# octavian-ganea/equidock_public

Hardware: NVIDIA H100
Metric: protein_pairs_per_sec_iegmn_fwd_kabsch (higher is better)
Workload: dtype f32

## Files before the change

### equidock_public_b200/_native.py

```python
from __future__ import annotations

import ctypes as C
import os

_HERE = os.path.dirname(os.path.abspath(__file__))
LIB_PATH = os.environ.get('EQD_LIB_PATH') or os.path.join(_HERE, 'libeqd_iegmn.so')

ABI_VERSION = 14
EDGE_FEATS, N_RBF, HID, H0, H0_PAD, N_RES_TYPES, HEADS, TILE_ROWS = 27, 15, 64, 69, 72, 21, 50, 128
STATUS_SVD_DEGENERATE, STATUS_NAN, STATUS_DEGREE_OVERFLOW, STATUS_BAD_RESIDUE = 1, 2, 4, 8

_vp, _i32, _f32 = C.c_void_p, C.c_int32, C.c_float


class EqdGraph(C.Structure):
    _fields_ = [('n_pairs', _i32), ('n_nodes', _i32), ('n_lig_nodes', _i32), ('n_edges', _i32),
                ('n_lig_edges', _i32), ('max_in_degree', _i32),
                ('seg_ptr', _vp), ('row_ptr', _vp), ('col_src', _vp), ('edge_dst', _vp),
                ('he_lig', _vp), ('he_rec', _vp),
                ('n_node_tiles', _i32), ('node_tiles', _vp)]


class EqdLayerParams(C.Structure):
    _fields_ = [('dh', _i32), ('dhp', _i32),
                ('w_proj', _vp), ('b_proj', _vp), ('w_edge1', _vp), ('edge_ln_g', _vp), ('edge_ln_b', _vp),
                ('w_edge2', _vp), ('b_edge2', _vp), ('w_coor1', _vp), ('b_coor1', _vp), ('w_coor2', _vp),
                ('b_coor2', _f32), ('w_edge_tc', _vp), ('w_node_tc', _vp), ('w_proj_tc', _vp),
                ('w_node1', _vp), ('b_node1', _vp), ('node_ln_g', _vp), ('node_ln_b', _vp),
                ('w_node2', _vp), ('b_node2', _vp),
                ('skip_weight_h', _f32), ('x_connection_init', _f32), ('leaky_slope', _f32), ('mma_products', _i32)]


class EqdLayerConsts(C.Structure):
    _fields_ = [('edge', _f32 * 64 * 5), ('node', _f32 * 304), ('proj_bias', _f32 * 320)]


class EqdDropout(C.Structure):
    _fields_ = [('seed', C.c_uint64), ('p', _f32), ('scale', _f32), ('threshold', C.c_uint32), ('layer', _i32),
                ('rank', _i32), ('reserved', _i32)]


def dropout_descriptor(p: float, seed: int, layer: int, rank: int = 0) -> EqdDropout:
    import numpy as np
    d = EqdDropout()
    d.seed, d.p, d.layer, d.rank = int(seed) & 0xFFFFFFFFFFFFFFFF, float(p), int(layer), int(rank)
    d.threshold = min(int(round(float(p) * 2.0 ** 32)), 0xFFFFFFFF)
    d.scale = 0.0 if p >= 1.0 else float(np.float32(1.0 / (1.0 - float(p))))
    return d


class EqdLayer(C.Structure):
    _fields_ = [('dev', EqdLayerParams), ('consts', EqdLayerConsts), ('dropout', EqdDropout)]


class EqdForwardIO(C.Structure):
    _fields_ = [(n, _vp) for n in ('emb', 'res_lig', 'res_rec', 'mu_lig', 'mu_rec', 'x_lig', 'x_rec', 'rot', 'trans',
                                   'ligand_out', 'sing', 'status', 'h_out', 'x_out', 'keypts', 'cov', 'ymean', 'stage_events',
                                   'train_stash')] + \
               [('train_stash_bytes', C.c_size_t)]


class EqdHeadParams(C.Structure):
    _fields_ = [('w_mean', _vp), ('b_mean', _vp), ('w_key', _vp), ('w_query', _vp), ('m_qk', _vp), ('leaky_slope', _f32)]


class EqdPairArchive(C.Structure):
    _fields_ = [('n_pairs', _i32)] + [(n, _vp) for n in (
        'lig_node_ptr', 'rec_node_ptr', 'lig_edge_ptr', 'rec_edge_ptr', 'pocket_ptr', 'lig_res_feat', 'rec_res_feat',
        'lig_x', 'rec_x', 'lig_mu_r_norm', 'rec_mu_r_norm', 'lig_src', 'lig_dst', 'rec_src', 'rec_dst', 'lig_he', 'rec_he',
        'lig_new_x', 'pocket_coors', 'bound_lig', 'bound_rec', 'lig_centroid')]


class EqdBatchOut(C.Structure):
    _fields_ = [(n, _vp) for n in ('res_feat', 'x', 'new_x', 'mu_r_norm', 'row_ptr', 'col_src', 'edge_dst', 'he_lig', 'he_rec',
                                   'seg_ptr',
                                   'node_tiles', 'pocket_ptr', 'pocket_lig', 'pocket_rec', 'bound_lig', 'bound_rec', 'rot',
                                   'trans')]


_G, _L, _H = C.POINTER(EqdGraph), C.POINTER(EqdLayer), C.POINTER(EqdHeadParams)
PROTOTYPES = {
    'eqd_abi_version': (C.c_int, []),
    'eqd_workspace_bytes': (C.c_size_t, [_i32, _i32, _i32]),
    'eqd_embed': (C.c_int, [_G, _vp, _vp, _vp, _vp, _vp, _vp, _vp, _vp, _vp, _vp]),
    'eqd_embed_checked': (C.c_int, [_G, _vp, _vp, _vp, _vp, _vp, _vp, _vp, _vp, _vp, _vp, _vp]),
    'eqd_project': (C.c_int, [_G, _L, _vp, _i32, _vp, _vp]),
    'eqd_edge_stage': (C.c_int, [_G, _L, _vp, _vp, _vp, _vp, _vp, _vp, _vp]),
    'eqd_edge_stage_ffma': (C.c_int, [_G, _L, _vp, _vp, _vp, _vp, _vp, _vp, _vp]),
    'eqd_node_stage': (C.c_int, [_G, _L, _L, _vp, _i32, _vp, _vp, _vp, _vp, _vp, _vp, _vp]),
    'eqd_kv_blocks_bytes': (C.c_size_t, [_i32]),
    'eqd_project_tc': (C.c_int, [_G, _L, _vp, _vp, _vp, _vp]),
    'eqd_project_tc0': (C.c_int, [_G, _L, _vp, _vp, _vp, _vp, _vp]),
    'eqd_attention_tc0': (C.c_int, [_G, _vp, _vp, _vp, _vp, _vp]),
    'eqd_node_mlp_tc0': (C.c_int, [_G, _L, _vp, _vp, _vp, _vp, _vp]),
    'eqd_node_stage_tc0': (C.c_int, [_G, _L, _L, _vp, _vp, _vp, _vp, _vp, _vp, _vp, _vp, _vp]),
    'eqd_kv_blocks': (C.c_int, [_G, _vp, _i32, _i32, _i32, _vp, _vp]),
    'eqd_attention_tc': (C.c_int, [_G, _vp, _vp, _vp, _vp]),
    'eqd_node_mlp_tc': (C.c_int, [_G, _L, _vp, _vp, _vp, _vp, _vp, _vp]),
    'eqd_node_stage_tc': (C.c_int, [_G, _L, _L, _vp, _vp, _vp, _vp, _vp, _vp, _vp, _vp, _vp]),
    'eqd_iegmn_layer_forward': (C.c_int, [_G, _L, _L, _vp, _i32, _vp, _vp, _vp, _vp, _vp, _vp, _vp, _vp, _vp, _vp,
                                          _vp]),
    'eqd_head_fold': (C.c_int, [_H, _vp, _vp]),
    'eqd_forward_workspace_bytes': (C.c_size_t, [_G]),
    'eqd_iegmn_forward': (C.c_int, [_G, C.POINTER(_L), _i32, _H, C.POINTER(EqdForwardIO), _vp, C.c_size_t, _vp]),
    'eqd_forward_stash_bytes': (C.c_size_t, [_G, _i32]),
    'eqd_forward_stash_offsets': (C.c_int, [_G, _i32, C.POINTER(C.c_size_t)]),
    'eqd_tn_partial_floats': (C.c_size_t, [C.c_int64, _i32, _i32, C.POINTER(_i32), C.POINTER(_i32)]),
    'eqd_tn_gemm': (C.c_int, [_vp, _i32, _i32, _vp, _i32, _i32, C.c_int64, _f32, _vp, _vp, C.POINTER(_i32), _vp]),
    'eqd_grad_reduce': (C.c_int, [_vp, _i32, C.c_int64, _vp, _vp, _i32, _vp, _vp]),
    'eqd_bwd_node_mlp': (C.c_int, [_G, _L] + [_vp] * 3 + [_i32, _vp, _vp, _i32] + [_vp] * 9 + [C.POINTER(_i32), _vp]),
    'eqd_bwd_attention': (C.c_int, [_G, _L, _vp, _vp, _i32, _vp, _vp, _vp, _vp]),
    'eqd_bwd_edge': (C.c_int, [_G, _L] + [_vp] * 14 + [C.POINTER(_i32), _vp]),
    'eqd_bwd_edge_gather': (C.c_int, [_G, _vp, _vp, _vp, _vp, _vp, _f32, _vp, _i32, _vp, _vp]),
    'eqd_bwd_project': (C.c_int, [_G, _L, _vp, _vp, _vp, _vp]),
    'eqd_bwd_embed': (C.c_int, [_G, _vp, _vp, _vp, _vp, _vp, _vp]),
    'eqd_bwd_head_workspace_bytes': (C.c_size_t, [_i32, _i32, _i32]),
    'eqd_bwd_head': (C.c_int, [_G, _H] + [_vp] * 9 + [C.c_size_t] + [_vp] * 6),
    'eqd_bwd_head_dropout': (C.c_int, [_G, _H, C.POINTER(EqdDropout)] + [_vp] * 9 + [C.c_size_t] + [_vp] * 6),
    'eqd_bwd_layer_inputs': (C.c_int, [_G, _L] + [_vp] * 5),
    'eqd_bwd_inputs': (C.c_int, [_G] + [_vp] * 11),
    'eqd_losses_workspace_bytes': (C.c_size_t, [_i32, _i32]),
    'eqd_losses': (C.c_int, [_G] + [_vp] * 7 + [_i32, _i32, _f32, _f32, _f32, _f32, _vp, C.c_size_t] + [_vp] * 6),
    'eqd_graph_build_workspace_bytes': (C.c_size_t, [_i32]),
    'eqd_graph_build_knn': (C.c_int, [_i32, _i32, _i32, _vp, _vp, _vp, _vp, _vp, _f32, _i32, _vp, C.c_size_t, _vp, _vp, _vp, _vp]),
    'eqd_graph_build_edges': (C.c_int, [_i32, _vp, _vp, _vp, _vp, _vp, _vp, _vp]),
    'eqd_assemble_batch': (C.c_int, [C.POINTER(EqdPairArchive), _i32, _vp, _i32, C.c_uint64, C.c_uint64, _i32, _f32, _i32,
                                     C.POINTER(EqdBatchOut), _vp]),
    'eqd_rmsd_meter': (C.c_int, [_G, _vp, _vp, _vp, _vp, _vp, _vp]),
    'eqd_sqnorm_partials': (C.c_int, [_vp, C.c_int64, _vp, _i32, _vp]),
    'eqd_clip_adam': (C.c_int, [_vp, _vp, _vp, _vp, C.c_int64, _vp, _i32, _f32, _f32, _f32, _f32, _f32, _f32, _i32, _f32, _vp, _vp]),
    'eqd_event_create': (_vp, []),
    'eqd_event_destroy': (None, [_vp]),
    'eqd_event_elapsed_ms': (C.c_float, [_vp, _vp]),
    'eqd_keypoints': (C.c_int, [_G, _H, _vp, _vp, _vp, C.c_size_t, _vp, _vp, _vp, _vp]),
    'eqd_keypoints_dropout': (C.c_int, [_G, _H, C.POINTER(EqdDropout), _vp, _vp, _vp, C.c_size_t, _vp, _vp, _vp, _vp]),
    'eqd_kabsch_apply': (C.c_int, [_G, _vp, _vp, _vp, _vp, _vp, _vp, _vp, _vp, _vp, _vp]),
}

_lib = None


class NativeLibraryError(RuntimeError):
    pass


def load():
    global _lib
    if _lib is not None:
        return _lib
    if not os.path.isfile(LIB_PATH):
        raise NativeLibraryError(
            f'{LIB_PATH} not found: build it with equidock_public_b200/csrc/build.sh '
            '(python -c "import __graft_entry__ as g; g.build()"). This engine has no CPU fallback.')
    lib = C.CDLL(LIB_PATH)
    for name, (res, args) in PROTOTYPES.items():
        fn = getattr(lib, name)
        fn.restype, fn.argtypes = res, args
    if lib.eqd_abi_version() != ABI_VERSION:
        raise NativeLibraryError(f'ABI mismatch: library {lib.eqd_abi_version()} vs binding {ABI_VERSION}')
    _lib = lib
    return lib


def check(rc: int, what: str):
    if rc == 0:
        return
    if rc <= -1000:
        raise NativeLibraryError(f'{what}: CUDA error {-(rc + 1000)} at kernel launch')
    names = {-1: 'EQD_ERR_BAD_ARG', -2: 'EQD_ERR_UNSUPPORTED', -3: 'EQD_ERR_WORKSPACE'}
    raise NativeLibraryError(f'{what}: {names.get(rc, rc)}')


def ptr(t):
    if t is None:
        return None
    return C.c_void_p(t.data_ptr())
```

### equidock_public_b200/csrc/edge_stage_tc.cu

```cuda
#include "tc_common.cuh"

namespace eqd {
#define TC_WGS 3
#define TC_THREADS (128 * TC_WGS)
#define TC_ROWS 64
#define TC_MAX_TN 32
#define TC_LD 72
#define TC_W_BYTES 67584
#define TC_W1_SPLIT 6144
#define TC_W23_BASE 18432
#define TC_W23_SPLIT 16384
#define TC_HE_FLOATS (TC_ROWS * EQD_EDGE_FEATS + 16)
#define TC_A_SPLIT 6144

struct __align__(128) TcWgSmem {
  unsigned char a[3 * TC_A_SPLIT];
  float msg[TC_ROWS * TC_LD];
  float he[TC_HE_FLOATS];
  double xs[2][TC_ROWS * 6];
  double xm[TC_ROWS * 3];
  double phi[TC_ROWS];
  int src[2][TC_ROWS];
  int dst[2][TC_ROWS];
  int rp[2][TC_MAX_TN + 4];
  unsigned long long he_bar;
};

struct EdgeConsts {
  float ln_g[64], ln_b[64], b2[64], b3[64], w4[64];
};

struct TcSmem {
  unsigned char w[TC_W_BYTES];
  TcWgSmem wg[TC_WGS];
  EdgeConsts cst;
  unsigned long long w_bar;
};

template <int P>
__global__ void __launch_bounds__(TC_THREADS, 1)
edge_stage_tc_kernel(eqd_graph g, eqd_layer_params p, const __grid_constant__ EdgeConsts cst_p,
                     const float* __restrict__ proj, const double* __restrict__ x_in, const double* __restrict__ x_orig,
                     float* __restrict__ aggr, double* __restrict__ x_out, int* __restrict__ status, int tn) {
  extern __shared__ __align__(128) unsigned char smem_raw[];
  TcSmem& S = *reinterpret_cast<TcSmem*>(smem_raw);
  const int tid = threadIdx.x, wgi = tid >> 7, t = tid & 127, r = t & 63, half = t >> 6;
  const int warp = t >> 5, lane = t & 31;
  TcWgSmem& W = S.wg[wgi];
  const EdgeConsts& cst = S.cst;
  const int bar = 1 + wgi;
  const int pw = 128 + 3 * p.dhp;
  const int ntiles = (g.n_nodes + tn - 1) / tn;
  const float slope = p.leaky_slope;

  if (tid == 0) {
    mbar_init(&S.w_bar, 1);
    for (int w = 0; w < TC_WGS; ++w) mbar_init(&S.wg[w].he_bar, 1);
    asm volatile("fence.mbarrier_init.release.cluster;" ::: "memory");
    mbar_expect_tx(&S.w_bar, TC_W_BYTES);
    bulk_g2s(S.w, p.w_edge_tc, TC_W_BYTES, &S.w_bar);
  }
  for (int i = tid; i < 5 * 64; i += TC_THREADS) (&S.cst.ln_g[0])[i] = (&cst_p.ln_g[0])[i];
  __syncthreads();
  mbar_wait(&S.w_bar, 0);
  unsigned he_phase = 0;
  const unsigned w_saddr = smem_u32(S.w), a_saddr = smem_u32(W.a);
  auto a_desc = [&](int sp, int kb) { return a_desc_at<TC_ROWS>(a_saddr, TC_A_SPLIT, 0, sp, kb); };

  auto prefetch = [&](int tile, int buf, int e0, int e1, int& off_l, int& n_l, int& off_r) {
    const int n0 = tile * tn, nn = min(tn, g.n_nodes - n0);
    const int ne = e1 - e0;
    off_l = off_r = 0;
    n_l = 0;
    if (ne <= TC_ROWS) {
      if (r < ne) {
        if (half == 0) cp_async4(&W.src[buf][r], g.col_src + e0 + r);
        else cp_async4(&W.dst[buf][r], g.edge_dst + e0 + r);
      }
      if (half == 0 && r <= nn) cp_async4(&W.rp[buf][r], g.row_ptr + n0 + r);
      const int el0 = min(e0, g.n_lig_edges), el1 = min(e1, g.n_lig_edges);
      n_l = el1 - el0;
      long sl = 0, sr = 0;
      unsigned bl = 0, br = 0;
      if (n_l > 0) {
        long b0 = (long)el0 * (EQD_EDGE_FEATS * 4), b1 = (long)el1 * (EQD_EDGE_FEATS * 4);
        sl = b0 & ~15L;
        bl = (unsigned)(((b1 + 15) & ~15L) - sl);
        off_l = (int)((b0 - sl) >> 2);
      }
      const int nr = ne - n_l;
      const unsigned dst_r_off = bl;
      if (nr > 0) {
        long b0 = (long)(e0 + n_l - g.n_lig_edges) * (EQD_EDGE_FEATS * 4), b1 = (long)(e1 - g.n_lig_edges) * (EQD_EDGE_FEATS * 4);
        sr = b0 & ~15L;
        br = (unsigned)(((b1 + 15) & ~15L) - sr);
        off_r = (int)(dst_r_off >> 2) + (int)((b0 - sr) >> 2);
      }
      if (t == 0) {
        mbar_expect_tx(&W.he_bar, bl + br);
        if (bl) bulk_g2s(W.he, reinterpret_cast<const unsigned char*>(g.he_lig) + sl, bl, &W.he_bar);
        if (br) bulk_g2s(reinterpret_cast<unsigned char*>(W.he) + dst_r_off, reinterpret_cast<const unsigned char*>(g.he_rec) + sr, br,
                         &W.he_bar);
      }
    }
    cp_async_commit();
  };
  auto prefetch_x = [&](int b, int ne_t) {
    if (r < ne_t && ne_t <= TC_ROWS) {
      const double* xp = x_in + (long)(half == 0 ? W.src[b][r] : W.dst[b][r]) * 3;
#pragma unroll
      for (int c = 0; c < 3; ++c) cp_async8(&W.xs[b][r * 6 + half * 3 + c], xp + c);
    }
    cp_async_commit();
  };
  auto row_range = [&](int tile, int& e0, int& e1) {
    const int n0 = tile * tn;
    e0 = __ldg(g.row_ptr + n0);
    e1 = __ldg(g.row_ptr + n0 + min(tn, g.n_nodes - n0));
  };

  int tile = blockIdx.x * TC_WGS + wgi;
  const int tstride = gridDim.x * TC_WGS;
  int buf = 0;
  int e0 = 0, ne = 0, off_l = 0, n_l = 0, off_r = 0;
  if (tile < ntiles) {
    int e1;
    row_range(tile, e0, e1);
    ne = e1 - e0;
    prefetch(tile, buf, e0, e1, off_l, n_l, off_r);
    cp_async_wait<0>();
    prefetch_x(buf, ne);
  }
  const int fr0 = warp * 16 + (lane >> 2), fc = 2 * (lane & 3);

  for (; tile < ntiles; tile += tstride) {
    const int n0 = tile * tn, nn = min(tn, g.n_nodes - n0);
    const bool has_next = tile + tstride < ntiles;
    int e0n = 0, e1n = 0, off_ln = 0, n_ln = 0, off_rn = 0;
    if (has_next) row_range(tile + tstride, e0n, e1n);
    const int nen = e1n - e0n;
    if (ne > TC_ROWS) {
      if (t == 0) atomicOr(status + g.n_pairs, EQD_STATUS_DEGREE_OVERFLOW);
      cp_async_wait<0>();
      wg_barrier(bar);
      if (has_next) {
        prefetch(tile + tstride, buf ^ 1, e0n, e1n, off_ln, n_ln, off_rn);
        cp_async_wait<0>();
        prefetch_x(buf ^ 1, nen);
      }
      e0 = e0n; ne = nen; off_l = off_ln; n_l = n_ln; off_r = off_rn; buf ^= 1;
      continue;
    }
    const int o_upd = 127 - t;
    const int nd_upd = o_upd / 3, comp_upd = o_upd - nd_upd * 3;
    const long gi_upd = (long)(n0 + nd_upd) * 3 + comp_upd;
    double xo_upd = 0.0, xi_upd = 0.0;
    if (o_upd < nn * 3) {
      xo_upd = x_orig[gi_upd];
      xi_upd = x_in[gi_upd];
    }
    cp_async_wait<0>();
    wg_barrier(bar);
    float2 ps[16], pd[16];
#pragma unroll
    for (int h = 0; h < 2; ++h) {
      const int fr = fr0 + 8 * h;
      const bool ok = fr < ne;
      const float* sp = proj + (long)(ok ? W.src[buf][fr] : 0) * pw + fc;
      const float* dp = proj + (long)(ok ? W.dst[buf][fr] : n0) * pw + 64 + fc;
#pragma unroll
      for (int j = 0; j < 8; ++j) {
        ps[2 * j + h] = __ldg(reinterpret_cast<const float2*>(sp + 8 * j));
        pd[2 * j + h] = __ldg(reinterpret_cast<const float2*>(dp + 8 * j));
      }
    }
    const bool valid = r < ne;
    {
      float a1v[24];
      mbar_wait(&W.he_bar, he_phase);
      he_phase ^= 1;
      const float* hrow = W.he + (r < n_l ? off_l + r * EQD_EDGE_FEATS : off_r + (r - n_l) * EQD_EDGE_FEATS);
      if (half == 0) {
#pragma unroll
        for (int k = 0; k < 24; ++k) a1v[k] = valid ? hrow[k] : 0.f;
      } else {
        double rx = 0.0, ry = 0.0, rz = 0.0;
        if (valid) {
          const double* xs = W.xs[buf] + r * 6;
          rx = xs[0] - xs[3];
          ry = xs[1] - xs[4];
          rz = xs[2] - xs[5];
          W.xm[r * 3 + 0] = rx;
          W.xm[r * 3 + 1] = ry;
          W.xm[r * 3 + 2] = rz;
        }
#pragma unroll
        for (int k = 0; k < 3; ++k) a1v[k] = valid ? hrow[24 + k] : 0.f;
        const float nd2 = valid ? -(float)(rx * rx + ry * ry + rz * rz) : -INFINITY;
        constexpr double kS[EQD_N_RBF] = {1.0, 1.5, 2.25, 3.375, 5.0625, 7.59375, 11.390625, 17.0859375, 25.62890625,
                                          38.443359375, 57.6650390625, 86.49755859375, 129.746337890625,
                                          194.6195068359375, 291.92926025390625};
#pragma unroll
        for (int j = 0; j < EQD_N_RBF; ++j)
          a1v[3 + j] = exp2f(nd2 * (float)(1.4426950408889634 / kS[j]));
#pragma unroll
        for (int k = 18; k < 24; ++k) a1v[k] = 0.f;
      }
      unsigned p0[12], p1[12], p2[12];
#pragma unroll
      for (int c = 0; c < 12; ++c) split3_pair<P>(a1v[2 * c], a1v[2 * c + 1], p0[c], p1[c], p2[c]);
#pragma unroll
      for (int j = 0; j < 3; ++j) a_store8<TC_ROWS, P>(W.a, TC_A_SPLIT, r, half * 24 + 8 * j, p0 + 4 * j, p1 + 4 * j, p2 + 4 * j);
    }
    tc_fence_before();
    const bool deg10 = wg_barrier_and(bar, t >= nn || W.rp[buf][t + 1] - W.rp[buf][t] == 10);
    unsigned af[3][4][4];
    {
      float v[32];
      wg_gemm6_issue<64, 0, P>(v, a_desc, [&](int sp, int kb) { return b_desc_ex(w_saddr + sp * TC_W1_SPLIT + kb * 2048, 1024, 128); },
                         3, false);
      if (has_next) prefetch(tile + tstride, buf ^ 1, e0n, e1n, off_ln, n_ln, off_rn);
      wg_mma_wait(v);
#pragma unroll
      for (int h = 0; h < 2; ++h)
#pragma unroll
        for (int j = 0; j < 8; ++j) {
          float& x0 = v[4 * j + 2 * h];
          float& x1 = v[4 * j + 2 * h + 1];
          x0 = __fadd_rn(__fadd_rn(x0, ps[2 * j + h].x), pd[2 * j + h].x);
          x1 = __fadd_rn(__fadd_rn(x1, ps[2 * j + h].y), pd[2 * j + h].y);
          x0 = fmaxf(x0, __fmul_rn(x0, slope));
          x1 = fmaxf(x1, __fmul_rn(x1, slope));
        }
      float pv[32];
#pragma unroll
      for (int i = 0; i < 32; ++i) pv[i] = __shfl_xor_sync(0xffffffffu, v[i], 2);
      float mean[2], rstd[2];
#pragma unroll
      for (int h = 0; h < 2; ++h) {
        float mh[2], qh[2];
#pragma unroll
        for (int ch = 0; ch < 2; ++ch) {
          float s0 = 0.f, s1 = 0.f;
#pragma unroll
          for (int c4 = 0; c4 < 8; ++c4) {
            s0 = __fadd_rn(s0, chain_val(v, pv, h, ch, c4, 0));
            s1 = __fadd_rn(s1, chain_val(v, pv, h, ch, c4, 1));
          }
          const float sp = s0 + s1;
          mh[ch] = (sp + __shfl_xor_sync(0xffffffffu, sp, 1)) * (1.f / 32.f);
          float q0 = 0.f, q1 = 0.f;
#pragma unroll
          for (int c4 = 0; c4 < 8; ++c4) {
            const float d0 = __fadd_rn(chain_val(v, pv, h, ch, c4, 0), -mh[ch]);
            const float d1 = __fadd_rn(chain_val(v, pv, h, ch, c4, 1), -mh[ch]);
            q0 = fmaf(d0, d0, q0);
            q1 = fmaf(d1, d1, q1);
          }
          const float qp = q0 + q1;
          qh[ch] = qp + __shfl_xor_sync(0xffffffffu, qp, 1);
        }
        const float m0 = mh[0], m1 = mh[1];
        mean[h] = 0.5f * (m0 + m1);
        const float dm = m0 - m1;
        const float var = (qh[0] + qh[1] + dm * dm * 16.f) * (1.f / 64.f);
        rstd[h] = 1.f / sqrtf(var + 1e-5f);
      }
#pragma unroll
      for (int j = 0; j < 8; ++j) {
        const float2 gj = *reinterpret_cast<const float2*>(&cst.ln_g[8 * j + fc]);
        const float2 bj = *reinterpret_cast<const float2*>(&cst.ln_b[8 * j + fc]);
#pragma unroll
        for (int h = 0; h < 2; ++h) {
          float& x0 = v[4 * j + 2 * h];
          float& x1 = v[4 * j + 2 * h + 1];
          x0 = fmaf(__fmul_rn(__fadd_rn(x0, -mean[h]), rstd[h]), gj.x, bj.x);
          x1 = fmaf(__fmul_rn(__fadd_rn(x1, -mean[h]), rstd[h]), gj.y, bj.y);
        }
      }
      acc_to_a_split3<4, P>(v, af);
    }
    if (has_next) {
      cp_async_wait<0>();
      prefetch_x(buf ^ 1, nen);
    }
    {
      auto w23 = [&](int hn) {
        return [&, hn](int sp, int kb) {
          return b_desc_ex(w_saddr + TC_W23_BASE + sp * TC_W23_SPLIT + kb * 4096 + hn * 1024, 2048, 128); };
      };
      float m[32], hd[32];
      wg_gemm6_rs_issue<64, 4, 0, false, P>(m, af, w23(0), false);
      wg_gemm6_rs_issue<64, 4, 0, false, P>(hd, af, w23(1), false);
      wg_mma_wait(m);
      wg_mma_wait(hd);
      float u[32];
#pragma unroll
      for (int j = 0; j < 8; ++j) {
        const float2 b2 = *reinterpret_cast<const float2*>(&cst.b2[8 * j + fc]);
        const float2 b3 = *reinterpret_cast<const float2*>(&cst.b3[8 * j + fc]);
#pragma unroll
        for (int h = 0; h < 2; ++h) {
          *reinterpret_cast<float2*>(W.msg + (fr0 + 8 * h) * TC_LD + 8 * j + fc) =
              make_float2(__fadd_rn(m[4 * j + 2 * h], b2.x), __fadd_rn(m[4 * j + 2 * h + 1], b2.y));
          const float x0 = __fadd_rn(hd[4 * j + 2 * h], b3.x), x1 = __fadd_rn(hd[4 * j + 2 * h + 1], b3.y);
          u[4 * j + 2 * h] = fmaxf(x0, __fmul_rn(x0, slope));
          u[4 * j + 2 * h + 1] = fmaxf(x1, __fmul_rn(x1, slope));
        }
      }
      float pu[32];
#pragma unroll
      for (int i = 0; i < 32; ++i) pu[i] = __shfl_xor_sync(0xffffffffu, u[i], 2);
      double phv[2];
#pragma unroll
      for (int h = 0; h < 2; ++h) {
        double red[2];
#pragma unroll
        for (int ch = 0; ch < 2; ++ch) {
          const float* w4 = cst.w4 + 32 * ch + 2 * (lane & 1);
          float p0 = 0.f, p1 = 0.f;
#pragma unroll
          for (int c4 = 0; c4 < 8; ++c4) {
            p0 = fmaf(chain_val(u, pu, h, ch, c4, 0), w4[4 * c4], p0);
            p1 = fmaf(chain_val(u, pu, h, ch, c4, 1), w4[4 * c4 + 1], p1);
          }
          const double pp = (double)p0 + (double)p1;
          red[ch] = pp + __shfl_xor_sync(0xffffffffu, pp, 1);
        }
        phv[h] = red[0] + red[1] + (double)p.b_coor2;
      }
      if ((lane & 3) == 0) {
        W.phi[fr0] = phv[0];
        W.phi[fr0 + 8] = phv[1];
      }
    }
    wg_barrier(bar);
    if (o_upd < nn * 3) {
      const int rs = W.rp[buf][nd_upd] - e0, re = W.rp[buf][nd_upd + 1] - e0;
      double sum = 0.0;
      if (deg10) {
#pragma unroll
        for (int j = 0; j < 10; ++j) {
          const int rr = nd_upd * 10 + j;
          sum += W.xm[rr * 3 + comp_upd] * W.phi[rr];
        }
      } else {
        for (int rr = rs; rr < re; ++rr) sum += W.xm[rr * 3 + comp_upd] * W.phi[rr];
      }
      const int deg = re - rs;
      const double upd = deg > 0 ? sum / (double)deg : 0.0;
      const double eta = (double)p.x_connection_init;
      x_out[gi_upd] = eta * xo_upd + (1.0 - eta) * xi_upd + upd;
    }
    {
      const int c = t & 63;
      const float* col = W.msg + c;
      if (deg10) {
        for (int nd = (nn * half) >> 1, nd1 = (nn * (half + 1)) >> 1; nd < nd1; ++nd) {
          const float* cr = col + nd * 10 * TC_LD;
          float s0 = 0.f, s1 = 0.f;
#pragma unroll
          for (int j = 0; j < 10; j += 2) {
            s0 += cr[j * TC_LD];
            s1 += cr[(j + 1) * TC_LD];
          }
          aggr[(long)(n0 + nd) * 64 + c] = (s0 + s1) / 10.f;
        }
      } else {
        for (int nd = (nn * half) >> 1, nd1 = (nn * (half + 1)) >> 1; nd < nd1; ++nd) {
          const int rs = W.rp[buf][nd] - e0, re = W.rp[buf][nd + 1] - e0;
          float s0 = 0.f, s1 = 0.f;
          int rr = rs;
          for (; rr + 1 < re; rr += 2) {
            s0 += col[rr * TC_LD];
            s1 += col[(rr + 1) * TC_LD];
          }
          if (rr < re) s0 += col[rr * TC_LD];
          aggr[(long)(n0 + nd) * 64 + c] = re > rs ? (s0 + s1) / (float)(re - rs) : 0.f;
        }
      }
    }
    e0 = e0n; ne = nen; off_l = off_ln; n_l = n_ln; off_r = off_rn; buf ^= 1;
  }
  cp_async_wait<0>();
  __syncthreads();
}

template <int P>
static int launch_edge_stage_tc(const eqd_graph* g, const eqd_layer* p_l, const float* proj, const double* x_in,
                                const double* x_orig, float* aggr, double* x_out, int32_t* status, int tn, void* stream) {
  const int ntiles = (g->n_nodes + tn - 1) / tn;
  EdgeConsts cst;
  memcpy(&cst, p_l->consts.edge, sizeof(cst));
  size_t smem = sizeof(TcSmem) + 128;
  EQD_SET_SMEM((edge_stage_tc_kernel<P>), smem);
  int grid = (ntiles + TC_WGS - 1) / TC_WGS;
  if (grid > EQD_SMS) grid = EQD_SMS;
  edge_stage_tc_kernel<P><<<grid, TC_THREADS, smem, (cudaStream_t)stream>>>(*g, p_l->dev, cst, proj, x_in, x_orig, aggr,
                                                                           x_out, status, tn);
  EQD_CUDA_LAUNCH_CHECK();
  return EQD_OK;
}

}

extern "C" int eqd_edge_stage(const eqd_graph* g, const eqd_layer* p_l, const float* proj, const double* x_in,
                              const double* x_orig, float* aggr, double* x_out, int32_t* status, void* stream) {
  const eqd_layer_params* p = p_l ? &p_l->dev : nullptr;
  if (!g || !p || !proj || !x_in || !x_orig || !aggr || !x_out || !status) return EQD_ERR_BAD_ARG;
  if (!p->w_edge_tc) return EQD_ERR_BAD_ARG;
  const int products = eqd_mma_products(p);
  if (!products) return EQD_ERR_UNSUPPORTED;
  if (g->max_in_degree < 1 || g->max_in_degree > EQD_TM) return EQD_ERR_UNSUPPORTED;
  if (!(p->leaky_slope >= 0.f && p->leaky_slope <= 1.f)) return EQD_ERR_UNSUPPORTED;
  if ((reinterpret_cast<uintptr_t>(g->he_lig) | reinterpret_cast<uintptr_t>(g->he_rec) |
       reinterpret_cast<uintptr_t>(p->w_edge_tc)) & 15)
    return EQD_ERR_BAD_ARG;
  if (g->max_in_degree > TC_ROWS || p_l->dropout.p > 0.f) return eqd_edge_stage_ffma(g, p_l, proj, x_in, x_orig, aggr, x_out, status, stream);
  if (g->n_nodes <= 0) return EQD_OK;
  int tn = TC_ROWS / g->max_in_degree;
  if (tn > TC_MAX_TN) tn = TC_MAX_TN;
  return products == 3 ? eqd::launch_edge_stage_tc<3>(g, p_l, proj, x_in, x_orig, aggr, x_out, status, tn, stream)
                       : eqd::launch_edge_stage_tc<6>(g, p_l, proj, x_in, x_orig, aggr, x_out, status, tn, stream);
}
```

### equidock_public_b200/csrc/forward.cu

```cuda
#include <cstdint>

#include "common.cuh"

namespace {

inline size_t al256(size_t v) { return (v + 255) & ~(size_t)255; }

struct Carve {
  size_t h0, x0, xa, xb, ha, hb, pa, pb, aggr, mu, kv, x5, head, keypts, ymean, cov, total;
  size_t kv_bytes, x5_rows, head_bytes;
};

Carve carve(const eqd_graph* g) {
  Carve c;
  const size_t N = (size_t)(g->n_nodes > 0 ? g->n_nodes : 0), B = (size_t)(g->n_pairs > 0 ? g->n_pairs : 0);
  size_t o = 0;
  auto take = [&](size_t bytes) { size_t at = o; o += al256(bytes); return at; };
  c.h0 = take(N * EQD_H0_PAD * 4);
  c.x0 = take(N * 3 * 8);
  c.xa = take(N * 3 * 8);
  c.xb = take(N * 3 * 8);
  c.ha = take(N * EQD_HID * 4);
  c.hb = take(N * EQD_HID * 4);
  c.pa = take(N * (128 + 3 * EQD_H0_PAD) * 4);
  c.pb = take(N * (128 + 3 * EQD_H0_PAD) * 4);
  c.aggr = take(N * EQD_HID * 4);
  c.mu = take(N * EQD_H0_PAD * 4);
  c.kv_bytes = eqd_kv_blocks_bytes(g->n_nodes);
  c.kv = take(c.kv_bytes);
  c.x5_rows = ((N + 7) / 8 + 8) * 8;
  c.x5 = take(c.x5_rows * 16 * 4);
  c.head_bytes = eqd_workspace_bytes(g->n_nodes, g->n_node_tiles, g->n_pairs);
  c.head = take(c.head_bytes);
  c.keypts = take(2 * B * EQD_HEADS * 3 * 8);
  c.ymean = take(2 * B * 3 * 8);
  c.cov = take(B * 9 * 8);
  c.total = o;
  return c;
}

}

extern "C" size_t eqd_forward_workspace_bytes(const eqd_graph* g) { return g ? carve(g).total : 0; }

namespace {
struct Stash {
  size_t h0, x, h, aggr, mu, total, x_stride, h_stride, a_stride, m_stride;
};
Stash stash_layout(const eqd_graph* g, int n_layers) {
  Stash s;
  const size_t N = (size_t)(g->n_nodes > 0 ? g->n_nodes : 0), L = (size_t)(n_layers > 0 ? n_layers : 0);
  s.x_stride = al256(N * 3 * 8);
  s.h_stride = al256(N * EQD_HID * 4);
  s.a_stride = al256(N * EQD_HID * 4);
  s.m_stride = al256(N * EQD_H0_PAD * 4);
  size_t o = 0;
  s.h0 = o; o += al256(N * EQD_H0_PAD * 4);
  s.x = o; o += L * s.x_stride;
  s.h = o; o += L * s.h_stride;
  s.aggr = o; o += L * s.a_stride;
  s.mu = o; o += L * s.m_stride;
  s.total = o;
  return s;
}
}

extern "C" size_t eqd_forward_stash_bytes(const eqd_graph* g, int32_t n_layers) { return g ? stash_layout(g, n_layers).total : 0; }
extern "C" int eqd_forward_stash_offsets(const eqd_graph* g, int32_t n_layers, size_t* out ) {
  if (!g || !out) return EQD_ERR_BAD_ARG;
  const Stash s = stash_layout(g, n_layers);
  out[0] = s.h0; out[1] = s.x; out[2] = s.x_stride; out[3] = s.h; out[4] = s.h_stride; out[5] = s.aggr; out[6] = s.a_stride;
  out[7] = s.mu; out[8] = s.m_stride;
  return EQD_OK;
}

extern "C" int eqd_iegmn_forward(const eqd_graph* g, const eqd_layer* const* layers, int32_t n_layers,
                                 const eqd_head_params* hp, const eqd_forward_io* io, void* workspace,
                                 size_t workspace_bytes, void* stream) {
  if (!g || !layers || n_layers < 1 || !hp || !io || !workspace) return EQD_ERR_BAD_ARG;
  if (!io->emb || !io->res_lig || !io->res_rec || !io->mu_lig || !io->mu_rec || !io->x_lig || !io->x_rec || !io->rot ||
      !io->trans || !io->ligand_out || !io->sing || !io->status || !io->h_out || !io->x_out)
    return EQD_ERR_BAD_ARG;
  if ((reinterpret_cast<uintptr_t>(io->h_out) | reinterpret_cast<uintptr_t>(io->x_out)) & 15)
    return EQD_ERR_BAD_ARG;
  for (int li = 0; li < n_layers; ++li)
    if (!layers[li]) return EQD_ERR_BAD_ARG;
  const Carve c = carve(g);
  if (workspace_bytes < c.total) return EQD_ERR_WORKSPACE;
  if (reinterpret_cast<uintptr_t>(workspace) & 255) return EQD_ERR_BAD_ARG;
  if (g->n_pairs <= 0 || g->n_nodes <= 0) return EQD_OK;
  cudaStream_t st = (cudaStream_t)stream;
  unsigned char* w = reinterpret_cast<unsigned char*>(workspace);
  float* h0 = reinterpret_cast<float*>(w + c.h0);
  double* x0 = reinterpret_cast<double*>(w + c.x0);
  double* xbuf[2] = {reinterpret_cast<double*>(w + c.xa), reinterpret_cast<double*>(w + c.xb)};
  float* hbuf[2] = {reinterpret_cast<float*>(w + c.ha), reinterpret_cast<float*>(w + c.hb)};
  float* pa = reinterpret_cast<float*>(w + c.pa);
  float* pb = reinterpret_cast<float*>(w + c.pb);
  float* aggr = reinterpret_cast<float*>(w + c.aggr);
  float* mu = reinterpret_cast<float*>(w + c.mu);
  unsigned char* kv = w + c.kv;
  float* x5 = reinterpret_cast<float*>(w + c.x5);
  double* keypts = io->keypts ? io->keypts : reinterpret_cast<double*>(w + c.keypts);
  double* ymean = io->ymean ? io->ymean : reinterpret_cast<double*>(w + c.ymean);
  double* cov = io->cov ? io->cov : reinterpret_cast<double*>(w + c.cov);
  const int N = g->n_nodes, B = g->n_pairs;
  unsigned char* sb = reinterpret_cast<unsigned char*>(io->train_stash);
  Stash sl;
  if (sb) {
    sl = stash_layout(g, n_layers);
    if (io->train_stash_bytes < sl.total || (reinterpret_cast<uintptr_t>(sb) & 255)) return EQD_ERR_WORKSPACE;
    h0 = reinterpret_cast<float*>(sb + sl.h0);
    x0 = reinterpret_cast<double*>(sb + sl.x);
  }

  const size_t plane = c.kv_bytes / 6, from = (size_t)(N / 8) * 1024;
  cudaError_t me = cudaSuccess;
  for (int pl = 0; pl < 6 && me == cudaSuccess; ++pl) me = cudaMemsetAsync(kv + pl * plane + from, 0, plane - from, st);
  if (me == cudaSuccess) me = cudaMemsetAsync(x5 + (size_t)N * 16, 0, (c.x5_rows - (size_t)N) * 16 * 4, st);
  if (me == cudaSuccess) me = cudaMemsetAsync(io->status, 0, (size_t)(B + 1) * sizeof(int32_t), st);
  if (me != cudaSuccess) return -(1000 + (int)me);
  auto stage_event = [&](int li, int which) {
    if (io->stage_events && io->stage_events[li * 4 + which]) cudaEventRecord((cudaEvent_t)io->stage_events[li * 4 + which], st);
  };
  int rc = eqd_embed_checked(g, io->emb, io->res_lig, io->res_rec, io->mu_lig, io->mu_rec, io->x_lig, io->x_rec, h0, x0,
                             io->status, stream);
  if (rc) return rc;
  const eqd_layer* l0_l = layers[0];
  const eqd_layer_params* l0 = &l0_l->dev;
  bool drop = false;
  for (int li = 0; li < n_layers; ++li) drop = drop || layers[li]->dropout.p > 0.f;
  const bool tc0 = l0->dh == EQD_H0 && l0->w_proj_tc && l0->w_node_tc && !drop;
  if (tc0) rc = eqd_project_tc0(g, l0_l, h0, pa, kv, x5, stream);
  else rc = eqd_project(g, l0_l, h0, l0->dh == EQD_H0 ? EQD_H0_PAD : EQD_HID, pa, stream);
  if (rc) return rc;
  const float* h_in = h0;
  int ldh = l0->dh == EQD_H0 ? EQD_H0_PAD : EQD_HID;
  const double* x_in = x0;
  for (int li = 0; li < n_layers; ++li) {
    const eqd_layer* lp_l = layers[li];
    const eqd_layer* lpn_l = li + 1 < n_layers ? layers[li + 1] : nullptr;
    const eqd_layer_params* lp = &lp_l->dev;
    const eqd_layer_params* lpn = lpn_l ? &lpn_l->dev : nullptr;
    const bool last = lpn == nullptr;
    float* h_out = last ? io->h_out : hbuf[li & 1];
    double* x_out = last ? io->x_out : xbuf[li & 1];
    if (sb) {
      if (!last) {
        h_out = reinterpret_cast<float*>(sb + sl.h + (size_t)(li + 1) * sl.h_stride);
        x_out = reinterpret_cast<double*>(sb + sl.x + (size_t)(li + 1) * sl.x_stride);
      }
      aggr = reinterpret_cast<float*>(sb + sl.aggr + (size_t)li * sl.a_stride);
      mu = reinterpret_cast<float*>(sb + sl.mu + (size_t)li * sl.m_stride);
    }
    stage_event(li, 0);
    rc = eqd_edge_stage(g, lp_l, pa, x_in, x0, aggr, x_out, io->status, stream);
    if (rc) return rc;
    stage_event(li, 1);
    stage_event(li, 2);
    if (lp->dh == EQD_HID && lp->w_node_tc && !drop && (!lpn || lpn->w_proj_tc)) {
      rc = eqd_node_stage_tc(g, lp_l, lpn_l, h_in, h0, pa, aggr, kv, mu, h_out, pb, stream);
    } else if (li == 0 && tc0 && (!lpn || lpn->w_proj_tc)) {
      rc = eqd_node_stage_tc0(g, lp_l, lpn_l, h0, pa, aggr, kv, x5, mu, h_out, pb, stream);
    } else {
      rc = eqd_node_stage(g, lp_l, lpn_l, h_in, ldh, h0, pa, aggr, sb ? mu : nullptr, h_out, pb, stream);
      if (!rc && lpn && lpn->dh == EQD_HID && lpn->w_node_tc && !drop) rc = eqd_kv_blocks(g, pb, 320, 192, 256, kv, stream);
    }
    if (rc) return rc;
    stage_event(li, 3);
    float* t = pa; pa = pb; pb = t;
    h_in = h_out;
    ldh = EQD_HID;
    x_in = x_out;
  }
  eqd_dropout head_drop = layers[n_layers - 1]->dropout;
  head_drop.layer = n_layers;
  rc = eqd_keypoints_dropout(g, hp, &head_drop, h_in, x_in, w + c.head, c.head_bytes, keypts, ymean, cov, stream);
  if (rc) return rc;
  return eqd_kabsch_apply(g, cov, ymean, io->x_lig, nullptr, io->rot, io->trans, io->ligand_out, io->sing, io->status, stream);
}

extern "C" void* eqd_event_create(void) {
  cudaEvent_t e = nullptr;
  return cudaEventCreate(&e) == cudaSuccess ? (void*)e : nullptr;
}
extern "C" void eqd_event_destroy(void* e) {
  if (e) cudaEventDestroy((cudaEvent_t)e);
}
extern "C" float eqd_event_elapsed_ms(void* a, void* b) {
  float ms = -1.f;
  if (!a || !b || cudaEventElapsedTime(&ms, (cudaEvent_t)a, (cudaEvent_t)b) != cudaSuccess) return -1.f;
  return ms;
}
```

### equidock_public_b200/csrc/node_mlp_tc.cu

```cuda
#include "tc_common.cuh"

namespace eqd {

#define NM_THREADS 256
#define NM_W5_SPLIT 34816
#define NM_W6_BASE 104448
#define NM_W6_SPLIT 8192
#define NM_W_BYTES 129024

struct NmConsts { float b5[64], ln_g[64], ln_b[64], b6[64]; };

#define NM_CHAINS 2
#define NM_SLOTS 3

struct NmSmem {
  unsigned char w[NM_W_BYTES];
  float stage[NM_CHAINS][NM_SLOTS][64 * 64];
  float c[256];
  unsigned long long w_bar;
};

template <int P>
__global__ void __launch_bounds__(NM_CHAINS * 128, 1)
node_mlp_tc_kernel(int n_nodes, eqd_layer_params p, const __grid_constant__ NmConsts cst, const float* __restrict__ h_in,
                   const float* __restrict__ aggr, const float* __restrict__ mu, const float* __restrict__ h0,
                   float* __restrict__ h_out) {
  extern __shared__ __align__(128) unsigned char smem_raw[];
  NmSmem& S = *reinterpret_cast<NmSmem*>(smem_raw);
  const int tid = threadIdx.x, wgi = tid >> 7, t = tid & 127, lane = t & 31;
  float (&ring)[NM_SLOTS][64 * 64] = S.stage[wgi];
  const int bar = 1 + wgi;
  const int ntiles = (n_nodes + 63) / 64, tstride = gridDim.x * NM_CHAINS, tile0 = blockIdx.x * NM_CHAINS + wgi;
  if (tid == 0) {
    mbar_init(&S.w_bar, 1);
    asm volatile("fence.mbarrier_init.release.cluster;" ::: "memory");
    mbar_expect_tx(&S.w_bar, NM_W_BYTES);
    bulk_g2s(S.w, p.w_node_tc, NM_W_BYTES, &S.w_bar);
  }
  for (int i = tid; i < 256; i += NM_CHAINS * 128) S.c[i] = reinterpret_cast<const float*>(&cst)[i];
  __syncthreads();
  const unsigned w_saddr = smem_u32(S.w);
  const float slope = p.leaky_slope, sk = p.skip_weight_h, sk1 = 1.f - p.skip_weight_h;
  const int fr0 = (t >> 5) * 16 + (lane >> 2), fc = 2 * (lane & 3);

  auto issue = [&](int q) {
    const int tile = tile0 + (q >> 2) * tstride, pc = q & 3;
    if (tile < ntiles) {
      const float* src = pc == 0 ? h_in : pc == 1 ? aggr : pc == 2 ? mu : h0;
      stage_rows64(ring[q % NM_SLOTS], src, pc == 3 ? EQD_H0_PAD : EQD_HID, 0, (long)tile * 64, min(64, n_nodes - tile * 64), t);
    } else {
      cp_async_commit();
    }
  };
  int q = 0;
  for (int i = 0; i < NM_SLOTS - 1; ++i) issue(i);
  mbar_wait(&S.w_bar, 0);

  for (int tile = tile0; tile < ntiles; tile += tstride) {
    const int node0 = tile * 64, nvalid = min(64, n_nodes - node0);
    float2 x4[2];
#pragma unroll
    for (int hh = 0; hh < 2; ++hh) {
      const int row = fr0 + 8 * hh;
      x4[hh] = row < nvalid ? *reinterpret_cast<const float2*>(h0 + (long)(node0 + row) * EQD_H0_PAD + 64 + fc)
                            : make_float2(0.f, 0.f);
    }
    float acc[32], hs[32];
#pragma unroll
    for (int j = 0; j < 8; ++j) {
      const float2 bj = *reinterpret_cast<const float2*>(&S.c[8 * j + fc]);
#pragma unroll
      for (int hh = 0; hh < 2; ++hh) {
        acc[4 * j + 2 * hh] = bj.x;
        acc[4 * j + 2 * hh + 1] = bj.y;
      }
    }
#pragma unroll 1
    for (int pc = 0; pc < 4; ++pc, ++q) {
      cp_async_wait<NM_SLOTS - 2>();
      wg_barrier(bar);
      issue(q + NM_SLOTS - 1);
      float v[32];
      staged_rows_to_frag(ring[q % NM_SLOTS], t, v);
      if (pc == 0) {
#pragma unroll
        for (int i = 0; i < 32; ++i) hs[i] = v[i];
      }
      unsigned af[3][4][4];
      acc_to_a_split3<4, P>(v, af);
      float d[32];
      wg_gemm6_rs_issue<64, 4, 0, false, P>(d, af, [&](int sp, int kb) {
        return b_desc_ex(w_saddr + (4 * pc + kb) * 2048 + sp * NM_W5_SPLIT, 1024, 128); }, false);
      wg_mma_wait(d);
#pragma unroll
      for (int i = 0; i < 32; ++i) acc[i] = __fadd_rn(acc[i], d[i]);
    }
    {
      unsigned a4[3][1][4];
#pragma unroll
      for (int hh = 0; hh < 2; ++hh) split3_pair<P>(x4[hh].x, x4[hh].y, a4[0][0][hh], a4[1][0][hh], a4[2][0][hh]);
#pragma unroll
      for (int sp = 0; sp < 3; ++sp) a4[sp][0][2] = a4[sp][0][3] = 0u;
      float d[32];
      wg_gemm6_rs_issue<64, 1, 0, false, P>(d, a4, [&](int sp, int kb) {
        return b_desc_ex(w_saddr + 16 * 2048 + sp * NM_W5_SPLIT, 1024, 128); }, false);
      wg_mma_wait(d);
#pragma unroll
      for (int i = 0; i < 32; ++i) acc[i] = __fadd_rn(acc[i], d[i]);
    }
    unsigned af[3][4][4];
    {
      float (&v)[32] = acc;
#pragma unroll
      for (int i = 0; i < 32; ++i) v[i] = fmaxf(v[i], __fmul_rn(v[i], slope));
      float pv[32];
#pragma unroll
      for (int i = 0; i < 32; ++i) pv[i] = __shfl_xor_sync(0xffffffffu, v[i], 2);
      float msum[2], rstd[2];
#pragma unroll
      for (int h = 0; h < 2; ++h) {
        float mh[2], qh[2];
#pragma unroll
        for (int ch = 0; ch < 2; ++ch) {
          float s0 = 0.f, s1 = 0.f;
#pragma unroll
          for (int c4 = 0; c4 < 8; ++c4) {
            s0 = __fadd_rn(s0, chain_val(v, pv, h, ch, c4, 0));
            s1 = __fadd_rn(s1, chain_val(v, pv, h, ch, c4, 1));
          }
          const float sp = __fadd_rn(s0, s1);
          mh[ch] = __fmul_rn(__fadd_rn(sp, __shfl_xor_sync(0xffffffffu, sp, 1)), 1.f / 32.f);
          float q0 = 0.f, q1 = 0.f;
#pragma unroll
          for (int c4 = 0; c4 < 8; ++c4) {
            const float d0 = __fadd_rn(chain_val(v, pv, h, ch, c4, 0), -mh[ch]);
            const float d1 = __fadd_rn(chain_val(v, pv, h, ch, c4, 1), -mh[ch]);
            q0 = __fmaf_rn(d0, d0, q0);
            q1 = __fmaf_rn(d1, d1, q1);
          }
          const float qp = __fadd_rn(q0, q1);
          qh[ch] = __fadd_rn(qp, __shfl_xor_sync(0xffffffffu, qp, 1));
        }
        msum[h] = __fadd_rn(mh[0], mh[1]);
        const float dm = __fadd_rn(mh[0], -mh[1]);
        const float var = __fmaf_rn(__fmul_rn(dm, dm), 16.f, __fadd_rn(qh[0], qh[1]));
        rstd[h] = 1.f / sqrtf(__fmaf_rn(var, 1.f / 64.f, 1e-5f));
      }
#pragma unroll
      for (int j = 0; j < 8; ++j) {
        const float2 gj = *reinterpret_cast<const float2*>(&S.c[64 + 8 * j + fc]);
        const float2 bj = *reinterpret_cast<const float2*>(&S.c[128 + 8 * j + fc]);
#pragma unroll
        for (int h = 0; h < 2; ++h) {
          float& x0 = v[4 * j + 2 * h];
          float& x1 = v[4 * j + 2 * h + 1];
          x0 = __fmaf_rn(__fmul_rn(__fmaf_rn(msum[h], -0.5f, x0), rstd[h]), gj.x, bj.x);
          x1 = __fmaf_rn(__fmul_rn(__fmaf_rn(msum[h], -0.5f, x1), rstd[h]), gj.y, bj.y);
        }
      }
      acc_to_a_split3<4, P>(v, af);
    }
    {
      float d[32];
      wg_gemm6_rs_issue<64, 4, 0, false, P>(d, af, [&](int sp, int kb) {
        return b_desc_ex(w_saddr + NM_W6_BASE + sp * NM_W6_SPLIT + kb * 2048, 1024, 128); }, false);
      wg_mma_wait(d);
#pragma unroll
      for (int hh = 0; hh < 2; ++hh) {
        const int row = fr0 + 8 * hh;
        if (row < nvalid) {
          float* o = h_out + (long)(node0 + row) * EQD_HID + fc;
#pragma unroll
          for (int j = 0; j < 8; ++j) {
            const float2 bj = *reinterpret_cast<const float2*>(&S.c[192 + 8 * j + fc]);
            const int i = 4 * j + 2 * hh;
            *reinterpret_cast<float2*>(o + 8 * j) =
                make_float2(__fmaf_rn(__fadd_rn(d[i], bj.x), sk, __fmul_rn(hs[i], sk1)),
                            __fmaf_rn(__fadd_rn(d[i + 1], bj.y), sk, __fmul_rn(hs[i + 1], sk1)));
          }
        }
      }
    }
  }
  cp_async_wait<0>();
}


#define NM0_W5_SPLIT 35840
#define NM0_W6_BASE 107520
#define NM0_W6_SPLIT 10240
#define NM0_W_BYTES 138240
#define NM0_A_SPLIT 20480
#define NM0_LD 84

struct Nm0Consts { float b5[80], ln_g[80], ln_b[80], b6[64]; };

struct Nm0Smem {
  unsigned char w[NM0_W_BYTES];
  unsigned char a[3 * NM0_A_SPLIT];
  float red[EQD_TM * 4];
  unsigned long long w_bar;
};

__global__ void __launch_bounds__(NM_THREADS, 1)
node_mlp0_tc_kernel(int n_nodes, eqd_layer_params p, const __grid_constant__ Nm0Consts cst, const float* __restrict__ h0,
                    const float* __restrict__ aggr, const float* __restrict__ mu , float* __restrict__ h_out) {
  extern __shared__ __align__(128) unsigned char smem_raw[];
  Nm0Smem& S = *reinterpret_cast<Nm0Smem*>(smem_raw);
  const int tid = threadIdx.x, q = tid, half = q >> 7, r = q & 127, wgi = tid >> 7;
  const int ntiles = (n_nodes + EQD_TM - 1) / EQD_TM;
  if (tid == 0) {
    mbar_init(&S.w_bar, 1);
    asm volatile("fence.mbarrier_init.release.cluster;" ::: "memory");
    mbar_expect_tx(&S.w_bar, NM0_W_BYTES);
    bulk_g2s(S.w, p.w_node_tc, NM0_W_BYTES, &S.w_bar);
  }
  __syncthreads();
  const unsigned w_saddr = smem_u32(S.w), a_saddr = smem_u32(S.a);
  float* const dtile = reinterpret_cast<float*>(S.a);
  auto a_desc = [&](int sp, int kb) { return a_desc_at<EQD_TM>(a_saddr, NM0_A_SPLIT, wgi, sp, kb); };
  mbar_wait(&S.w_bar, 0);
  const float slope = p.leaky_slope;
  float* red = S.red;

  for (int tile = blockIdx.x; tile < ntiles; tile += gridDim.x) {
    const int node = tile * EQD_TM + r;
    const bool valid = node < n_nodes;
    auto row32 = [&](const float* base, int ld, float (&v)[32]) {
      const float4* sp = reinterpret_cast<const float4*>(base + (long)node * ld + half * 32);
#pragma unroll
      for (int c4 = 0; c4 < 8; ++c4) {
        float4 t = valid ? sp[c4] : make_float4(0.f, 0.f, 0.f, 0.f);
        v[c4 * 4] = t.x; v[c4 * 4 + 1] = t.y; v[c4 * 4 + 2] = t.z; v[c4 * 4 + 3] = t.w;
      }
    };
    auto extra8 = [&](const float* base) {
      if (half == 0) {
        const float4* ep = reinterpret_cast<const float4*>(base + (long)node * EQD_H0_PAD + 64);
        float4 a = valid ? ep[0] : make_float4(0.f, 0.f, 0.f, 0.f), b = valid ? ep[1] : make_float4(0.f, 0.f, 0.f, 0.f);
        float t[8] = {a.x, a.y, a.z, a.w, b.x, b.y, b.z, b.w};
        store_extra8_split3<EQD_TM>(S.a, NM0_A_SPLIT, r, 64, t);
      }
    };
    float acc[32], accx[16];
#pragma unroll
    for (int c = 0; c < 32; ++c) acc[c] = cst.b5[half * 32 + c];
#pragma unroll
    for (int c = 0; c < 16; ++c) accx[c] = cst.b5[64 + c];
    auto piece = [&](int kb0, int nkb) {
      tc_fence_before();
      __syncthreads();
      {
        float d[40];
        wg_gemm6<80>(d, a_desc, [&](int sp, int kb) {
          return b_desc_ex(w_saddr + (kb0 + kb) * (80 * 32) + sp * NM0_W5_SPLIT, 80 * 16, 128); }, nkb, false);
        __syncthreads();
        wg_store_d<80>(dtile + wgi * 64 * NM0_LD, NM0_LD, d, tid & 127);
      }
      __syncthreads();
      const float* dr = dtile + r * NM0_LD;
#pragma unroll
      for (int c = 0; c < 32; ++c) acc[c] += dr[half * 32 + c];
      if (half == 0) {
#pragma unroll
        for (int c = 0; c < 16; ++c) accx[c] += dr[64 + c];
      }
      __syncthreads();
    };
    {
      float v[32];
      row32(h0, EQD_H0_PAD, v);
      store_half_split3<EQD_TM>(S.a, NM0_A_SPLIT, r, half * 32, v);
      extra8(h0);
      piece(0, 5);
      row32(aggr, EQD_HID, v);
      store_half_split3<EQD_TM>(S.a, NM0_A_SPLIT, r, half * 32, v);
      piece(5, 4);
      row32(mu, EQD_H0_PAD, v);
      store_half_split3<EQD_TM>(S.a, NM0_A_SPLIT, r, half * 32, v);
      extra8(mu);
      piece(9, 5);
    }
    {
      const int nh = half == 0 ? 37 : 32;
      float sum = 0.f;
#pragma unroll
      for (int c = 0; c < 32; ++c) {
        acc[c] = lrelu(acc[c], slope);
        sum += acc[c];
      }
      if (half == 0) {
#pragma unroll
        for (int c = 0; c < 5; ++c) {
          accx[c] = lrelu(accx[c], slope);
          sum += accx[c];
        }
      }
      const float mh = sum / (float)nh;
      float m2 = 0.f;
#pragma unroll
      for (int c = 0; c < 32; ++c) {
        float d = acc[c] - mh;
        m2 = fmaf(d, d, m2);
      }
      if (half == 0) {
#pragma unroll
        for (int c = 0; c < 5; ++c) {
          float d = accx[c] - mh;
          m2 = fmaf(d, d, m2);
        }
      }
      red[(r * 2 + half) * 2 + 0] = mh;
      red[(r * 2 + half) * 2 + 1] = m2;
      __syncthreads();
      const float m0 = red[r * 4 + 0], m1 = red[r * 4 + 2];
      const float mean = (37.f * m0 + 32.f * m1) * (1.f / 69.f);
      const float dm = m0 - m1;
      const float var = (red[r * 4 + 1] + red[r * 4 + 3] + dm * dm * (37.f * 32.f / 69.f)) * (1.f / 69.f);
      const float rstd = 1.f / sqrtf(var + 1e-5f);
#pragma unroll
      for (int c = 0; c < 32; ++c) acc[c] = (acc[c] - mean) * rstd * cst.ln_g[half * 32 + c] + cst.ln_b[half * 32 + c];
      store_half_split3<EQD_TM>(S.a, NM0_A_SPLIT, r, half * 32, acc);
      if (half == 0) {
        float t[8];
#pragma unroll
        for (int c = 0; c < 5; ++c) t[c] = (accx[c] - mean) * rstd * cst.ln_g[64 + c] + cst.ln_b[64 + c];
        t[5] = t[6] = t[7] = 0.f;
        store_extra8_split3<EQD_TM>(S.a, NM0_A_SPLIT, r, 64, t);
      }
    }
    tc_fence_before();
    __syncthreads();
    {
      float d[32];
      wg_gemm6<64>(d, a_desc, [&](int sp, int kb) {
        return b_desc_ex(w_saddr + NM0_W6_BASE + sp * NM0_W6_SPLIT + kb * 2048, 1024, 128); }, 5, false);
      __syncthreads();
      wg_store_d<64>(dtile + wgi * 64 * NM0_LD, NM0_LD, d, tid & 127);
    }
    __syncthreads();
    {
      float v[32];
      tile_ld32f(dtile, NM0_LD, r, half * 32, v);
#pragma unroll
      for (int c = 0; c < 32; ++c) v[c] += cst.b6[half * 32 + c];
      if (valid) {
        float4* o = reinterpret_cast<float4*>(h_out + (long)node * EQD_HID + half * 32);
#pragma unroll
        for (int c4 = 0; c4 < 8; ++c4) o[c4] = make_float4(v[c4 * 4], v[c4 * 4 + 1], v[c4 * 4 + 2], v[c4 * 4 + 3]);
      }
    }
    __syncthreads();
  }
}

template <int P>
static int launch_node_mlp_tc(const eqd_graph* g, const eqd_layer* p_l, const float* h_in, const float* aggr,
                              const float* mu, const float* h0, float* h_out, void* stream) {
  NmConsts cst;
  memcpy(&cst, p_l->consts.node, sizeof(cst));
  const int ntiles = (g->n_nodes + 63) / 64;
  const size_t smem = sizeof(NmSmem) + 128;
  EQD_SET_SMEM(node_mlp_tc_kernel<P>, smem);
  int grid = (ntiles + NM_CHAINS - 1) / NM_CHAINS;
  if (grid > EQD_SMS) grid = EQD_SMS;
  node_mlp_tc_kernel<P><<<grid, NM_CHAINS * 128, smem, (cudaStream_t)stream>>>(g->n_nodes, p_l->dev, cst, h_in, aggr, mu,
                                                                             h0, h_out);
  EQD_CUDA_LAUNCH_CHECK();
  return EQD_OK;
}

}

extern "C" int eqd_node_mlp_tc(const eqd_graph* g, const eqd_layer* p_l, const float* h_in, const float* aggr,
                               const float* mu, const float* h0, float* h_out, void* stream) {
  const eqd_layer_params* p = p_l ? &p_l->dev : nullptr;
  if (!g || !p || !h_in || !aggr || !mu || !h0 || !h_out) return EQD_ERR_BAD_ARG;
  if (p_l->dropout.p > 0.f) return EQD_ERR_UNSUPPORTED;
  if (p->dh != 64 || p->dhp != 64) return EQD_ERR_UNSUPPORTED;
  if (!(p->leaky_slope >= 0.f && p->leaky_slope <= 1.f)) return EQD_ERR_UNSUPPORTED;
  const int products = eqd_mma_products(p);
  if (!products) return EQD_ERR_UNSUPPORTED;
  if (!p->w_node_tc || (reinterpret_cast<uintptr_t>(p->w_node_tc) & 15)) return EQD_ERR_BAD_ARG;
  if (g->n_nodes <= 0) return EQD_OK;
  return products == 3 ? eqd::launch_node_mlp_tc<3>(g, p_l, h_in, aggr, mu, h0, h_out, stream)
                       : eqd::launch_node_mlp_tc<6>(g, p_l, h_in, aggr, mu, h0, h_out, stream);
}

extern "C" int eqd_node_mlp_tc0(const eqd_graph* g, const eqd_layer* p_l, const float* h0, const float* aggr,
                                const float* mu, float* h_out, void* stream) {
  const eqd_layer_params* p = p_l ? &p_l->dev : nullptr;
  if (!g || !p || !h0 || !aggr || !mu || !h_out) return EQD_ERR_BAD_ARG;
  if (p_l->dropout.p > 0.f) return EQD_ERR_UNSUPPORTED;
  if (p->dh != 69 || p->dhp != 72 || !eqd_mma_products(p)) return EQD_ERR_UNSUPPORTED;
  if (!(p->leaky_slope >= 0.f && p->leaky_slope <= 1.f)) return EQD_ERR_UNSUPPORTED;
  if (!p->w_node_tc || (reinterpret_cast<uintptr_t>(p->w_node_tc) & 15)) return EQD_ERR_BAD_ARG;
  if (g->n_nodes <= 0) return EQD_OK;
  eqd::Nm0Consts cst;
  memcpy(&cst, p_l->consts.node, sizeof(cst));
  int ntiles = (g->n_nodes + EQD_TM - 1) / EQD_TM;
  size_t smem = sizeof(eqd::Nm0Smem) + 128;
  EQD_SET_SMEM((eqd::node_mlp0_tc_kernel), smem);
  int grid = ntiles < EQD_SMS ? ntiles : EQD_SMS;
  eqd::node_mlp0_tc_kernel<<<grid, NM_THREADS, smem, (cudaStream_t)stream>>>(g->n_nodes, *p, cst, h0, aggr, mu, h_out);
  EQD_CUDA_LAUNCH_CHECK();
  return EQD_OK;
}

extern "C" int eqd_attention_tc0(const eqd_graph*, const float*, const void*, const float*, float*, void*);

extern "C" int eqd_node_stage_tc0(const eqd_graph* g, const eqd_layer* p_l, const eqd_layer* p_next_l,
                                  const float* h0, const float* proj, const float* aggr, void* kv, const float* x5,
                                  float* mu, float* h_out, float* proj_next, void* stream) {
  const eqd_layer_params* p = p_l ? &p_l->dev : nullptr;
  const eqd_layer_params* p_next = p_next_l ? &p_next_l->dev : nullptr;
  if (!g || !p || !kv || !mu || !x5) return EQD_ERR_BAD_ARG;
  if (p_next && !proj_next) return EQD_ERR_BAD_ARG;
  if (!eqd_mma_products(p)) return EQD_ERR_UNSUPPORTED;
  int rc = eqd_attention_tc0(g, proj, kv, x5, mu, stream);
  if (rc) return rc;
  rc = eqd_node_mlp_tc0(g, p_l, h0, aggr, mu, h_out, stream);
  if (rc) return rc;
  if (p_next) rc = eqd_project_tc(g, p_next_l, h_out, proj_next, kv, stream);
  return rc;
}

extern "C" int eqd_project_tc(const eqd_graph*, const eqd_layer*, const float*, float*, void*, void*);
int eqd_attention_tc_products(const eqd_graph*, const float*, const void*, float*, int, void*);


extern "C" int eqd_node_stage_tc(const eqd_graph* g, const eqd_layer* p_l, const eqd_layer* p_next_l,
                                 const float* h_in, const float* h0, const float* proj, const float* aggr, void* kv,
                                 float* mu, float* h_out, float* proj_next, void* stream) {
  const eqd_layer_params* p = p_l ? &p_l->dev : nullptr;
  const eqd_layer_params* p_next = p_next_l ? &p_next_l->dev : nullptr;
  if (!g || !p || !kv || !mu) return EQD_ERR_BAD_ARG;
  if (p_next && !proj_next) return EQD_ERR_BAD_ARG;
  const int products = eqd_mma_products(p);
  if (!products) return EQD_ERR_UNSUPPORTED;
  int rc = eqd_attention_tc_products(g, proj, kv, mu, products, stream);
  if (rc) return rc;
  rc = eqd_node_mlp_tc(g, p_l, h_in, aggr, mu, h0, h_out, stream);
  if (rc) return rc;
  if (p_next) rc = eqd_project_tc(g, p_next_l, h_out, proj_next, kv, stream);
  return rc;
}
```

### equidock_public_b200/engine.py

```python
from __future__ import annotations

import ctypes as C
import sys
import threading
from typing import Dict, List, Optional, Sequence

import numpy as np
import torch

from . import _native as nat
from .hetero_graph import LIGAND, LL, RECEPTOR, RR


def _dev_f32(t, device):
    return t.detach().to(device=device, dtype=torch.float32).contiguous()


def _host_f32(t):
    return t.detach().to(device='cpu', dtype=torch.float32).contiguous()


def _upload_blob(tensors: Dict[str, torch.Tensor], device) -> Dict[str, torch.Tensor]:
    offs, total = {}, 0
    for k, t in tensors.items():
        offs[k] = total
        total += (t.numel() * t.element_size() + 255) & ~255
    host = torch.zeros(max(total, 256), dtype=torch.uint8)
    for k, t in tensors.items():
        n = t.numel() * t.element_size()
        host[offs[k]:offs[k] + n] = t.contiguous().view(-1).view(torch.uint8)
    dev = host.to(device)
    out = {}
    for k, t in tensors.items():
        n = t.numel() * t.element_size()
        out[k] = dev[offs[k]:offs[k] + n].view(t.dtype).view(t.shape)
    out['_blob'] = dev
    return out


def umma_bf16x3(w: torch.Tensor) -> torch.Tensor:
    n, k = w.shape
    assert n % 8 == 0 and k % 8 == 0
    parts, r = [], w.to(torch.float32)
    for _ in range(3):
        b = r.to(torch.bfloat16)
        parts.append(b)
        r = r - b.to(torch.float32)
    out = [b.reshape(n // 8, 8, k // 8, 8).permute(2, 0, 1, 3).contiguous().reshape(-1) for b in parts]
    return torch.cat(out)


_PY_FORWARD = False

PRECISIONS = {'fp32': 0, 'bf16x3': 3}


def draw_dropout(p: float, rank: int = 0):
    if not p > 0:
        return None
    seed = int(torch.empty((), dtype=torch.int64).random_(-2 ** 63, 2 ** 63 - 1)) & 0xFFFFFFFFFFFFFFFF
    return float(p), seed, int(rank)


def with_dropout(descs, dropout, first_layer: int = 0):
    if dropout is None:
        return list(descs)
    p, seed, rank = dropout
    out = []
    for li, d in enumerate(descs):
        c = nat.EqdLayer.from_buffer_copy(d)
        c.dropout = nat.dropout_descriptor(p, seed, first_layer + li, rank)
        out.append(c)
    return out


def head_dropout(dropout, n_layers: int):
    return None if dropout is None else nat.dropout_descriptor(dropout[0], dropout[1], n_layers, dropout[2])


def check_precision(precision: str) -> str:
    if precision not in PRECISIONS:
        raise ValueError(f'precision must be one of {sorted(PRECISIONS)}, got {precision!r}')
    return precision


class PackedLayer:

    def __init__(self, sd: Dict[str, torch.Tensor], device, skip_weight_h: float, x_connection_init: float,
                 leaky_slope: float):
        f = lambda k: _host_f32(sd[k])
        w1, b1 = f('edge_mlp.0.weight'), f('edge_mlp.0.bias')
        wq, wk, wv = f('att_mlp_Q.0.weight'), f('att_mlp_K.0.weight'), f('att_mlp_V.0.weight')
        w5, b5 = f('node_mlp.0.weight'), f('node_mlp.0.bias')
        w6, b6 = f('node_mlp.4.weight'), f('node_mlp.4.bias')
        dh = int(wq.shape[0])
        if dh not in (nat.HID, nat.H0):
            raise ValueError(f'IEGMN layer width {dh} is not supported by the CUDA engine (64 or 69)')
        dhp = nat.HID if dh == nat.HID else nat.H0_PAD
        n_e = nat.EDGE_FEATS + nat.N_RBF
        assert w1.shape == (nat.HID, 2 * dh + n_e) and w5.shape == (dh, 2 * dh + nat.HID + nat.H0)
        z = lambda *s: torch.zeros(*s, dtype=torch.float32)
        pw = 128 + 3 * dhp
        w_proj, b_proj = z(dhp, pw), z(pw)
        w_proj[:dh, 0:64] = w1[:, 0:dh].t()
        w_proj[:dh, 64:128] = w1[:, dh:2 * dh].t()
        w_proj[:dh, 128:128 + dh] = wq.t()
        w_proj[:dh, 128 + dhp:128 + dhp + dh] = wk.t()
        w_proj[:dh, 128 + 2 * dhp:128 + 2 * dhp + dh] = wv.t()
        b_proj[64:128] = b1
        w_edge1 = z(44, 64)
        w_edge1[:n_e] = w1[:, 2 * dh:].t()
        w_node1 = z(2 * dhp + 64 + nat.H0_PAD, dhp)
        w_node1[0:dh, :dh] = w5[:, 0:dh].t()
        w_node1[dhp:dhp + 64, :dh] = w5[:, dh:dh + 64].t()
        w_node1[dhp + 64:dhp + 64 + dh, :dh] = w5[:, dh + 64:2 * dh + 64].t()
        w_node1[2 * dhp + 64:2 * dhp + 64 + nat.H0, :dh] = w5[:, 2 * dh + 64:].t()
        pad = lambda v: torch.cat([v, z(dhp - dh)]) if dhp > dh else v.clone()
        w_node2 = z(dhp, 64)
        w_node2[:dh] = w6.t()
        self.dh, self.dhp = dh, dhp
        w1e = z(64, 48)
        w1e[:, :n_e] = w1[:, 2 * dh:]
        w2d, w3d = f('edge_mlp.4.weight').double(), f('coors_mlp.0.weight').double()
        w32 = (w3d @ w2d).float()
        b32 = (w3d @ f('edge_mlp.4.bias').double() + f('coors_mlp.0.bias').double()).float()
        w_edge_tc = torch.cat([umma_bf16x3(w1e), umma_bf16x3(torch.cat([f('edge_mlp.4.weight'), w32]))]).contiguous()
        assert w_edge_tc.numel() * 2 == 67584
        self.edge_consts_host = torch.stack([f('edge_mlp.3.weight'), f('edge_mlp.3.bias'), f('edge_mlp.4.bias'),
                                             b32, f('coors_mlp.4.weight').reshape(-1)]).cpu().contiguous()
        tc = {}
        self.node_consts_host = self.proj_bias_host = None
        if dh == nat.HID:
            w5p = z(64, 272)
            w5p[:, :261] = w5
            tc['w_node_tc'] = torch.cat([umma_bf16x3(w5p), umma_bf16x3(w6)]).contiguous()
            groups = [w1[:, 0:64], w1[:, 64:128], wq, wk, wv]
            tc['w_proj_tc'] = torch.cat([umma_bf16x3(gw.contiguous()) for gw in groups]).contiguous()
            assert tc['w_node_tc'].numel() * 2 == 129024 and tc['w_proj_tc'].numel() * 2 == 122880
            self.node_consts_host = torch.stack([b5, f('node_mlp.3.weight'), f('node_mlp.3.bias'), b6]).cpu().contiguous()
            self.proj_bias_host = b_proj.cpu().contiguous()
        else:
            p80 = lambda w: torch.cat([w, z(w.shape[0], 80 - w.shape[1])], 1)
            x16 = z(16, 69)
            x16[0:4], x16[4:8], x16[8], x16[9], x16[10:15] = wk[64:68], wv[64:68], wk[68], wv[68], wq[64:69]
            groups = [w1[:, 0:69], w1[:, 69:138], wq[0:64], wk[0:64], wv[0:64], x16]
            tc['w_proj_tc'] = torch.cat([umma_bf16x3(p80(gw).contiguous()) for gw in groups]).contiguous()
            w5p = z(80, 224)
            w5p[:69, 0:69] = (w5[:, 0:69].double() + w5[:, 202:271].double()).float()
            w5p[:69, 80:144] = w5[:, 69:133]
            w5p[:69, 144:213] = w5[:, 133:202]
            tc['w_node_tc'] = torch.cat([umma_bf16x3(w5p), umma_bf16x3(p80(w6).contiguous())]).contiguous()
            assert tc['w_proj_tc'].numel() * 2 == 161280 and tc['w_node_tc'].numel() * 2 == 138240
            p80v = lambda v: torch.cat([v, z(80 - v.shape[0])])
            self.node_consts_host = torch.cat([p80v(b5), p80v(f('node_mlp.3.weight')), p80v(f('node_mlp.3.bias')), b6]).cpu().contiguous()
            pb = z(320)
            pb[64:128] = b1
            self.proj_bias_host = pb.cpu().contiguous()
        self.t = _upload_blob({
            **tc,
            'w_proj': w_proj, 'b_proj': b_proj, 'w_edge1': w_edge1,
            'edge_ln_g': f('edge_mlp.3.weight'), 'edge_ln_b': f('edge_mlp.3.bias'),
            'w_edge2': f('edge_mlp.4.weight').t().contiguous(), 'b_edge2': f('edge_mlp.4.bias'),
            'w_coor1': f('coors_mlp.0.weight').t().contiguous(), 'b_coor1': f('coors_mlp.0.bias'),
            'w_coor2': f('coors_mlp.4.weight').reshape(-1).contiguous(),
            'w_node1': w_node1, 'b_node1': pad(b5),
            'node_ln_g': pad(f('node_mlp.3.weight')), 'node_ln_b': pad(f('node_mlp.3.bias')),
            'w_node2': w_node2, 'b_node2': b6, 'w_edge_tc': w_edge_tc,
        }, device)
        lay = nat.EqdLayer()
        s = lay.dev
        s.dh, s.dhp = dh, dhp
        for k, v in self.t.items():
            if not k.startswith('_'):
                setattr(s, k, v.data_ptr())
        for name, host in (('edge', self.edge_consts_host), ('node', self.node_consts_host), ('proj_bias', self.proj_bias_host)):
            if host is not None:
                flat = host.reshape(-1).numpy()
                C.memmove(C.addressof(getattr(lay.consts, name)), flat.ctypes.data, flat.nbytes)
        s.b_coor2 = float(sd['coors_mlp.4.bias'].detach().reshape(-1)[0].item())
        s.skip_weight_h, s.x_connection_init, s.leaky_slope = skip_weight_h, x_connection_init, leaky_slope
        self.struct = lay
        self._descriptors = {}

    def descriptor(self, mma_products: int = 0):
        if mma_products == 0 or self.dh != nat.HID:
            return self.struct
        src, d = self._descriptors.get(mma_products, (None, None))
        if src is not self.struct:
            d = nat.EqdLayer.from_buffer_copy(self.struct)
            d.dev.mma_products = mma_products
            self._descriptors[mma_products] = (self.struct, d)
        return d


class PackedHead:

    def __init__(self, w_mean, b_mean, w_key, w_query, device, leaky_slope: float):
        dev = torch.device(device)
        inplace = all(t.is_cuda and t.device == dev and t.dtype == torch.float32 and t.is_contiguous() and t.data_ptr() % 16 == 0
                      for t in (b_mean, w_key, w_query)) and w_mean.is_cuda
        if inplace:
            self.t = {'w_mean': w_mean.detach().to(torch.float32).t().contiguous(), 'b_mean': b_mean.detach(),
                      'w_key': w_key.detach(), 'w_query': w_query.detach()}
        else:
            self.t = _upload_blob({'w_mean': _host_f32(w_mean).t().contiguous(), 'b_mean': _host_f32(b_mean),
                                   'w_key': _host_f32(w_key), 'w_query': _host_f32(w_query)}, device)
        assert self.t['w_key'].shape == (nat.HEADS * nat.HID, nat.HID)
        s = nat.EqdHeadParams()
        for k, v in self.t.items():
            if not k.startswith('_'):
                setattr(s, k, v.data_ptr())
        s.leaky_slope = leaky_slope
        self.struct = s
        self.m_qk = torch.empty(nat.HEADS, nat.HID, nat.HID, dtype=torch.float64, device=device)
        with torch.cuda.device(device):
            nat.check(nat.load().eqd_head_fold(C.byref(s), self.m_qk.data_ptr(), torch.cuda.current_stream().cuda_stream),
                      'eqd_head_fold')
        s.m_qk = self.m_qk.data_ptr()


def _aligned_he(he, device):
    he = he.to(device=device, dtype=torch.float32).contiguous()
    nbytes = he.numel() * 4
    try:
        room = he.untyped_storage().nbytes() - he.storage_offset() * 4
    except RuntimeError:
        room = nbytes
    if he.data_ptr() % 16 == 0 and room >= ((nbytes + 15) & ~15):
        return he
    buf = torch.empty(((nbytes + 15) // 16) * 4 + 4, dtype=torch.float32, device=device)
    own = buf[:he.numel()].view(he.shape)
    own.copy_(he)
    return own


def node_tiles_for(n_lig: Sequence[int], n_rec: Sequence[int], device):
    seg = np.zeros(len(n_lig) + len(n_rec) + 1, dtype=np.int64)
    seg[1:] = np.cumsum(np.asarray(list(n_lig) + list(n_rec), dtype=np.int64))
    tiles = [(s, n0) for s in range(len(seg) - 1) for n0 in range(int(seg[s]), int(seg[s + 1]), nat.TILE_ROWS)]
    small = torch.from_numpy(np.concatenate([seg.astype(np.int32), np.asarray(tiles, dtype=np.int32).reshape(-1)]))
    small = small.to(device, non_blocking=True)
    return seg, small[:len(seg)], small[len(seg):]


class GraphPlan:

    def __init__(self, n_lig: Sequence[int], n_rec: Sequence[int], src_l, dst_l, src_r, dst_r, he_l, he_r,
                 device, max_in_degree: int = 10):
        assert len(n_lig) == len(n_rec) and len(n_lig) > 0
        N_l = sum(int(v) for v in n_lig)
        N = N_l + sum(int(v) for v in n_rec)
        i32 = dict(dtype=torch.int32, device=device)
        src_l, dst_l = src_l.to(**i32), dst_l.to(**i32)
        src_r, dst_r = src_r.to(**i32), dst_r.to(**i32)
        E_l, E = int(src_l.shape[0]), int(src_l.shape[0]) + int(src_r.shape[0])
        col_src = torch.cat([src_l, src_r + N_l]).contiguous()
        edge_dst = torch.cat([dst_l, dst_r + N_l]).contiguous()
        d64 = edge_dst.long()
        unsorted = (d64[1:] < d64[:-1]).any() if E > 1 else None
        row_ptr = torch.searchsorted(edge_dst, torch.arange(N + 1, **i32), out_int32=True).contiguous()
        he_l, he_r = _aligned_he(he_l, device), _aligned_he(he_r, device)
        assert he_l.shape == (E_l, nat.EDGE_FEATS) and he_r.shape == (E - E_l, nat.EDGE_FEATS)
        self._finish(n_lig, n_rec, E_l, E, E_l, col_src, edge_dst, row_ptr, he_l, he_r, *node_tiles_for(n_lig, n_rec, device),
                     device, max_in_degree, unsorted)

    def _finish(self, n_lig, n_rec, E_l, E, n_lig_edges, col_src, edge_dst, row_ptr, he_l, he_r, seg_ptr_host, seg_ptr,
                node_tiles, device, max_in_degree, unsorted=None, keep=()):
        self.n_pairs = len(n_lig)
        self.forward_ws_bytes = None
        self.n_lig_list, self.n_rec_list = [int(v) for v in n_lig], [int(v) for v in n_rec]
        self.N_l, self.N_r = sum(self.n_lig_list), sum(self.n_rec_list)
        self.N = self.N_l + self.N_r
        self.device = device
        self.E_l, self.E_r, self.E = int(E_l), int(E) - int(E_l), int(E)
        self.col_src, self.edge_dst, self.row_ptr = col_src, edge_dst, row_ptr
        self.unsorted = unsorted if unsorted is not None else torch.zeros((), dtype=torch.bool, device=device)
        self.unsorted_i32 = self.unsorted.to(torch.int32).reshape(1)
        self._arange = None
        self.he_l, self.he_r = he_l, he_r
        self.edge_perm = None
        self.seg_ptr_host, self.seg_ptr, self.node_tiles = seg_ptr_host, seg_ptr, node_tiles
        self.n_node_tiles = int(node_tiles.numel()) // 2
        self._keep = keep
        g = nat.EqdGraph()
        g.n_pairs, g.n_nodes, g.n_lig_nodes = self.n_pairs, self.N, self.N_l
        g.n_edges, g.n_lig_edges, g.max_in_degree = self.E, int(n_lig_edges), int(max_in_degree)
        g.seg_ptr, g.row_ptr = seg_ptr.data_ptr(), row_ptr.data_ptr()
        g.col_src, g.edge_dst = col_src.data_ptr(), edge_dst.data_ptr()
        g.he_lig, g.he_rec = he_l.data_ptr(), he_r.data_ptr()
        g.n_node_tiles, g.node_tiles = self.n_node_tiles, node_tiles.data_ptr()
        self.struct = g

    def refresh(self, graph) -> bool:
        n_l = [int(v) for v in graph.batch_num_nodes(LIGAND).tolist()]
        n_r = [int(v) for v in graph.batch_num_nodes(RECEPTOR).tolist()]
        src_l, dst_l = graph.edges(etype=LL)
        src_r, dst_r = graph.edges(etype=RR)
        if (n_l != self.n_lig_list or n_r != self.n_rec_list or int(src_l.shape[0]) != self.E_l
                or int(src_r.shape[0]) != self.E_r):
            return False
        E_l = self.E_l
        self.col_src[:E_l].copy_(src_l)
        torch.add(src_r, self.N_l, out=self.col_src[E_l:])
        self.edge_dst[:E_l].copy_(dst_l)
        torch.add(dst_r, self.N_l, out=self.edge_dst[E_l:])
        if self.E > 1:
            torch.any(self.edge_dst[1:] < self.edge_dst[:-1], dim=0, keepdim=True, out=self.unsorted.view(1))
        self.unsorted_i32.copy_(self.unsorted.view(1))
        if self._arange is None:
            self._arange = torch.arange(self.N + 1, dtype=torch.int32, device=self.device)
        torch.searchsorted(self.edge_dst, self._arange, out_int32=True, out=self.row_ptr)
        for own, new in ((self.he_l, graph.edges[LL].data['he']), (self.he_r, graph.edges[RR].data['he'])):
            if own.data_ptr() != new.data_ptr():
                own.copy_(new)
        return True

    @classmethod
    def from_device_arrays(cls, n_lig: Sequence[int], n_rec: Sequence[int], E_l: int, E: int, col_src, edge_dst, row_ptr,
                           he_l, he_r, seg_ptr, node_tiles, seg_ptr_host, device, max_in_degree: int = 10, keep=()) -> 'GraphPlan':
        plan = object.__new__(cls)
        plan._finish(n_lig, n_rec, E_l, E, E if he_r is he_l else E_l, col_src, edge_dst, row_ptr, he_l, he_r, seg_ptr_host,
                     seg_ptr, node_tiles, device, max_in_degree, keep=keep)
        return plan

    @classmethod
    def from_graph(cls, graph, device, max_in_degree: int = 10, he=None, sort: bool = False) -> 'GraphPlan':
        n_l = graph.batch_num_nodes(LIGAND).tolist()
        n_r = graph.batch_num_nodes(RECEPTOR).tolist()
        he_l, he_r = he if he is not None else (graph.edges[LL].data['he'], graph.edges[RR].data['he'])
        sides = [(*graph.edges(etype=LL), he_l), (*graph.edges(etype=RR), he_r)]
        perms = None
        if sort:
            sides = [tuple(t.to(device) for t in side) for side in sides]
            perms = tuple(torch.sort(d.long(), stable=True).indices for _, d, _ in sides)
            sides = [tuple(t[perm] for t in side) for side, perm in zip(sides, perms)]
        (src_l, dst_l, he_l), (src_r, dst_r, he_r) = sides
        plan = cls(n_l, n_r, src_l, dst_l, src_r, dst_r, he_l, he_r, device, max_in_degree)
        plan.edge_perm = perms
        return plan

    def caller_edge_order(self, dhe):
        dhe_l, dhe_r = dhe[:self.E_l], dhe[self.E_l:self.E]
        if self.edge_perm is not None:
            dhe_l = torch.empty_like(dhe_l).index_copy_(0, self.edge_perm[0].to(dhe.device), dhe_l)
            dhe_r = torch.empty_like(dhe_r).index_copy_(0, self.edge_perm[1].to(dhe.device), dhe_r)
        return dhe_l, dhe_r


def plan_for(graph, device, max_in_degree, sort: bool = False) -> GraphPlan:
    cached = getattr(graph, '_eqd_plan', None)
    if not sort and cached is not None and cached.device == device and cached.struct.max_in_degree == max_in_degree:
        return cached
    plan = GraphPlan.from_graph(graph, device, max_in_degree, sort=sort)
    try:
        graph._eqd_plan = plan
    except AttributeError:
        pass
    return plan


def retry_sorted(graph, plan: GraphPlan, run):
    try:
        return run(plan)
    except UnsortedEdges:
        return run(plan_for(graph, plan.device, plan.struct.max_in_degree, sort=True))


class _StatusPool:

    def __init__(self):
        self.free, self.lock = [], threading.Lock()

    def take(self, n: int) -> torch.Tensor:
        with self.lock:
            for i, b in enumerate(self.free):
                if b.numel() >= n:
                    return self.free.pop(i)
        return torch.empty(max(n, 1024), dtype=torch.int32, pin_memory=True)

    def give(self, buf: torch.Tensor):
        with self.lock:
            if len(self.free) < 64:
                self.free.append(buf)


_STATUS_POOL = _StatusPool()


class _StatusLease:

    def __init__(self, n):
        self.buf, self.n = _STATUS_POOL.take(n), n

    def view(self):
        return self.buf[:self.n]

    def release(self):
        if self.buf is not None:
            _STATUS_POOL.give(self.buf)
            self.buf = None

    def __del__(self):
        try:
            self.release()
        except Exception:
            pass


class NativeStageTimer:

    def __init__(self):
        self.lib, self.sets, self.spare = nat.load(), [], []

    def reserve(self, n_forwards, n_layers):
        for _ in range(n_forwards):
            self.spare.append((C.c_void_p * (4 * n_layers))(*[self.lib.eqd_event_create() for _ in range(4 * n_layers)]))

    def new_forward(self, n_layers):
        if self.spare and len(self.spare[-1]) == 4 * n_layers:
            arr = self.spare.pop()
        else:
            arr = (C.c_void_p * (4 * n_layers))(*[self.lib.eqd_event_create() for _ in range(4 * n_layers)])
        self.sets.append(arr)
        return arr

    def _pairs(self, name):
        off = 0 if name == 'edge_stage' else 2
        for arr in self.sets:
            for li in range(len(arr) // 4):
                yield arr[li * 4 + off], arr[li * 4 + off + 1]

    def mean_ms(self, name):
        v = [self.lib.eqd_event_elapsed_ms(a, b) for a, b in self._pairs(name)]
        v = [x for x in v if x >= 0]
        return float(np.mean(v)) if v else None

    def total_ms(self, name):
        return float(sum(x for x in (self.lib.eqd_event_elapsed_ms(a, b) for a, b in self._pairs(name)) if x >= 0))

    def close(self):
        for arr in self.sets + self.spare:
            for e in arr:
                self.lib.eqd_event_destroy(e)
        self.sets, self.spare = [], []


class IEGMNEngine:

    @staticmethod
    def launches_per_forward(n_layers: int) -> int:
        n = 2 + 7
        for li in range(n_layers):
            last = li == n_layers - 1
            n += 1 + 2 + (0 if last else 1)
        return n

    def __init__(self, device):
        self.device = torch.device(device)
        if self.device.type != 'cuda':
            raise nat.NativeLibraryError('the IEGMN engine runs on a CUDA device only (no CPU fallback)')
        self.lib = nat.load()

    def forward(self, plan: GraphPlan, emb: torch.Tensor, layers: List[PackedLayer], head: PackedHead,
                res_l, res_r, mu_l, mu_r, x_l, x_r, check_status: bool = True, log=None,
                stage_timer=None, record_event: bool = True, train_stash=None,
                mma_products: int = 0, dropout=None) -> Dict[str, torch.Tensor]:
        with torch.cuda.device(self.device):
            lib, dev = self.lib, self.device
            st = C.c_void_p(torch.cuda.current_stream(dev).cuda_stream)
            N, B = plan.N, plan.n_pairs
            f32 = dict(dtype=torch.float32, device=dev)
            f64 = dict(dtype=torch.float64, device=dev)
            cf = lambda t: t.to(**f32).contiguous()
            res_l, res_r, mu_l, mu_r, x_l, x_r = map(cf, (res_l, res_r, mu_l, mu_r, x_l, x_r))
            assert x_l.shape == (plan.N_l, 3) and x_r.shape == (plan.N_r, 3)
            g = C.byref(plan.struct)
            if plan.forward_ws_bytes is None:
                plan.forward_ws_bytes = int(lib.eqd_forward_workspace_bytes(g))
            ws = torch.empty(plan.forward_ws_bytes, dtype=torch.uint8, device=dev)
            rot, trans = torch.empty(B, 3, 3, **f32), torch.empty(B, 1, 3, **f32)
            lig_out, h_fin = torch.empty(plan.N_l, 3, **f32), torch.empty(N, nat.HID, **f32)
            sing, x_fin = torch.empty(B, 3, **f64), torch.empty(N, 3, **f64)
            keyp = torch.empty(2 * B, nat.HEADS, 3, **f64)
            cov, ymean = torch.empty(B, 9, **f64), torch.empty(2 * B, 3, **f64)
            status = torch.empty(B + 1, dtype=torch.int32, device=dev)
            io = nat.EqdForwardIO()
            for name, t in (('emb', emb), ('res_lig', res_l), ('res_rec', res_r), ('mu_lig', mu_l), ('mu_rec', mu_r),
                            ('x_lig', x_l), ('x_rec', x_r), ('rot', rot), ('trans', trans), ('ligand_out', lig_out),
                            ('sing', sing), ('status', status), ('h_out', h_fin), ('x_out', x_fin), ('keypts', keyp),
                            ('cov', cov), ('ymean', ymean)):
                setattr(io, name, t.data_ptr())
            if train_stash is not None:
                io.train_stash, io.train_stash_bytes = train_stash.data_ptr(), int(train_stash.numel())
            events = stage_timer.new_forward(len(layers)) if stage_timer is not None else None
            io.stage_events = C.cast(events, C.c_void_p) if events is not None else None
            descs = with_dropout([l.descriptor(mma_products) for l in layers], dropout)
            larr = (C.POINTER(nat.EqdLayer) * len(layers))(*[C.pointer(d) for d in descs])
            nat.check(lib.eqd_iegmn_forward(g, larr, len(layers), C.byref(head.struct), C.byref(io), nat.ptr(ws),
                                            plan.forward_ws_bytes, st), 'eqd_iegmn_forward')
            kab = lambda mask: nat.check(lib.eqd_kabsch_apply(
                g, nat.ptr(cov), nat.ptr(ymean), nat.ptr(x_l), nat.ptr(mask), nat.ptr(rot), nat.ptr(trans),
                nat.ptr(lig_out), nat.ptr(sing), nat.ptr(status), st), 'eqd_kabsch_apply')
            lease = _StatusLease(B + 2)
            status_host = lease.view()
            status_host[:B + 1].copy_(status, non_blocking=True)
            status_host[B + 1:].copy_(plan.unsorted_i32, non_blocking=True)
            status_event = None
            if record_event:
                status_event = torch.cuda.Event()
                status_event.record()
            out = {'status_lease': lease, 'ligand_coors': lig_out, 'keypts': keyp, 'rotation': rot,
                   'translation': trans, 'h': h_fin, 'x64': x_fin, 'cov': cov, 'sing': sing, 'status': status,
                   'unsorted': plan.unsorted, 'kabsch': kab, 'status_host': status_host, 'status_event': status_event, '_keep': (ws, ymean, x_l)}
            if dropout is not None:
                out.update(dropout_layers=descs, dropout_head=head_dropout(dropout, len(layers)))
            if check_status:
                self.resolve_status(plan, out, kab, log)
            return out

    def resolve_status(self, plan: GraphPlan, out, kab, log=None):
        with torch.cuda.device(self.device):
            try:
                self._resolve_status(plan, out, kab, log)
            finally:
                lease = out.get('status_lease')
                if lease is not None:
                    out['status_host'] = out['status_host'].clone()
                    lease.release()

    def _resolve_status(self, plan: GraphPlan, out, kab, log=None):
        out['status_event'].synchronize()
        st_host = out['status_host']
        if int(st_host[-1]) != 0:
            raise UnsortedEdges()
        if int(st_host[plan.n_pairs]) & nat.STATUS_BAD_RESIDUE:
            raise IndexError('res_feat holds a residue index outside [0, 21): index out of range in self '
                             '(nn.Embedding, rigid_docking_model.py:460)')
        if int(st_host[plan.n_pairs]) & nat.STATUS_DEGREE_OVERFLOW:
            raise nat.NativeLibraryError(
                f'a node has more than max_in_degree={plan.struct.max_in_degree} in-edges; '
                'pass the true bound (args["graph_max_neighbor"])')
        pair_st = st_host[:plan.n_pairs]
        if not bool(pair_st.any()):
            return
        if bool((pair_st & nat.STATUS_NAN).any()):
            raise AssertionError('NaN in the Kabsch covariance (rigid_docking_model.py:570)')
        eye_idx = torch.tensor([0, 4, 8], device=self.device)
        for b in torch.nonzero(pair_st & nat.STATUS_SVD_DEGENERATE).reshape(-1).tolist():
            mask = torch.zeros(plan.n_pairs, dtype=torch.int32, device=self.device)
            mask[b] = 1
            num_it = 0
            while True:
                noise = torch.rand(3, 3)
                out['cov'][b, eye_idx] += torch.diagonal(noise).to(self.device, torch.float64)
                kab(mask)
                num_it += 1
                if num_it > 10:
                    if log is not None:
                        log('SVD consistently numerically unstable! Exitting ... ')
                    sys.exit(1)
                if int(out['status'][b].item()) & nat.STATUS_SVD_DEGENERATE == 0:
                    break


def run_layer(plan: GraphPlan, lay: PackedLayer, desc, inputs, keep_mu: bool):
    x_l, h_l, h0_l, _, xo_l, x_r, h_r, h0_r, _, xo_r = inputs
    dev = x_l.device
    lib = IEGMNEngine(dev).lib
    N, dhp = plan.N, lay.dhp
    f32, f64 = dict(dtype=torch.float32, device=dev), dict(dtype=torch.float64, device=dev)
    h = torch.zeros(N, dhp, **f32)
    h[:, :lay.dh] = torch.cat([h_l, h_r]).to(**f32)
    h0 = torch.zeros(N, nat.H0_PAD, **f32)
    h0[:, :nat.H0] = torch.cat([h0_l, h0_r]).to(**f32)
    x_in = torch.cat([x_l, x_r]).to(**f64).contiguous()
    x_orig = torch.cat([xo_l, xo_r]).to(**f64).contiguous()
    proj = torch.empty(N, 128 + 3 * dhp, **f32)
    aggr, h_out = torch.empty(N, nat.HID, **f32), torch.empty(N, nat.HID, **f32)
    mu = torch.empty(N, dhp, **f32) if keep_mu else None
    x_out = torch.empty(N, 3, **f64)
    status = torch.zeros(plan.n_pairs + 1, dtype=torch.int32, device=dev)
    with torch.cuda.device(dev):
        st = C.c_void_p(torch.cuda.current_stream(dev).cuda_stream)
        g, lp = C.byref(plan.struct), C.byref(desc)
        nat.check(lib.eqd_project(g, lp, nat.ptr(h), dhp, nat.ptr(proj), st), 'eqd_project')
        nat.check(lib.eqd_iegmn_layer_forward(g, lp, None, nat.ptr(h), dhp, nat.ptr(h0), nat.ptr(x_in),
                                              nat.ptr(x_orig), nat.ptr(proj), None, nat.ptr(aggr), nat.ptr(mu),
                                              nat.ptr(h_out), nat.ptr(x_out), nat.ptr(status), st),
                  'eqd_iegmn_layer_forward')
    if int(status[plan.n_pairs].item()) & nat.STATUS_DEGREE_OVERFLOW:
        raise nat.NativeLibraryError(f'IEGMN_Layer.forward: in-degree above {plan.struct.max_in_degree}')
    return h, h0, x_in, aggr, mu, h_out, x_out


class UnsortedEdges(RuntimeError):
    pass
```

### include/eqd_iegmn.h

```cpp
#ifndef EQD_IEGMN_H
#define EQD_IEGMN_H

#include <stddef.h>
#include <stdint.h>

#ifdef __cplusplus
extern "C" {
#endif

#define EQD_ABI_VERSION 14

#define EQD_EDGE_FEATS 27
#define EQD_N_RBF 15
#define EQD_HID 64
#define EQD_H0 69
#define EQD_H0_PAD 72
#define EQD_N_RES_TYPES 21
#define EQD_HEADS 50
#define EQD_TILE_ROWS 128

enum {
  EQD_OK = 0,
  EQD_ERR_BAD_ARG = -1,
  EQD_ERR_UNSUPPORTED = -2,
  EQD_ERR_WORKSPACE = -3
};

#define EQD_STATUS_SVD_DEGENERATE 1
#define EQD_STATUS_NAN 2
#define EQD_STATUS_DEGREE_OVERFLOW 4
#define EQD_STATUS_BAD_RESIDUE 8

typedef struct eqd_graph {
  int32_t n_pairs;
  int32_t n_nodes;
  int32_t n_lig_nodes;
  int32_t n_edges;
  int32_t n_lig_edges;
  int32_t max_in_degree;
  const int32_t* seg_ptr;
  const int32_t* row_ptr;
  const int32_t* col_src;
  const int32_t* edge_dst;
  const float* he_lig;
  const float* he_rec;
  int32_t n_node_tiles;
  const int32_t* node_tiles;
} eqd_graph;

typedef struct eqd_layer_params {
  int32_t dh, dhp;
  const float* w_proj;
  const float* b_proj;
  const float* w_edge1;
  const float* edge_ln_g;
  const float* edge_ln_b;
  const float* w_edge2;
  const float* b_edge2;
  const float* w_coor1;
  const float* b_coor1;
  const float* w_coor2;
  float b_coor2;
  const void* w_edge_tc;
  const void* w_node_tc;
  const void* w_proj_tc;
  const float* w_node1;
  const float* b_node1;
  const float* node_ln_g;
  const float* node_ln_b;
  const float* w_node2;
  const float* b_node2;
  float skip_weight_h;
  float x_connection_init;
  float leaky_slope;
  int32_t mma_products;
} eqd_layer_params;

typedef struct eqd_layer_consts {
  float edge[5][64];
  float node[304];
  float proj_bias[320];
} eqd_layer_consts;

typedef struct eqd_dropout {
  uint64_t seed;
  float p;
  float scale;
  uint32_t threshold;
  int32_t layer;
  int32_t rank;
  int32_t reserved;
} eqd_dropout;

typedef struct eqd_layer {
  eqd_layer_params dev;
  eqd_layer_consts consts;
  eqd_dropout dropout;
} eqd_layer;

typedef struct eqd_head_params {
  const float* w_mean;
  const float* b_mean;
  const float* w_key;
  const float* w_query;
  const double* m_qk;
  float leaky_slope;
} eqd_head_params;

int eqd_abi_version(void);

size_t eqd_workspace_bytes(int32_t n_nodes, int32_t n_node_tiles, int32_t n_pairs);

int eqd_embed(const eqd_graph* g, const float* emb ,
              const float* res_feat_lig, const float* res_feat_rec,
              const float* mu_lig, const float* mu_rec,
              const float* x_lig , const float* x_rec ,
              float* h0, double* x64, void* stream);
int eqd_embed_checked(const eqd_graph* g, const float* emb, const float* res_feat_lig, const float* res_feat_rec,
                      const float* mu_lig, const float* mu_rec, const float* x_lig, const float* x_rec,
                      float* h0, double* x64, int32_t* status , void* stream);

int eqd_project(const eqd_graph* g, const eqd_layer* p, const float* h, int32_t ldh,
                float* proj, void* stream);

int eqd_edge_stage(const eqd_graph* g, const eqd_layer* p, const float* proj,
                   const double* x_in, const double* x_orig, float* aggr, double* x_out,
                   int32_t* status , void* stream);

int eqd_edge_stage_ffma(const eqd_graph* g, const eqd_layer* p, const float* proj,
                        const double* x_in, const double* x_orig, float* aggr, double* x_out,
                        int32_t* status , void* stream);

int eqd_node_stage(const eqd_graph* g, const eqd_layer* p, const eqd_layer* p_next,
                   const float* h_in, int32_t ldh, const float* h0, const float* proj,
                   const float* aggr, float* mu, float* h_out, float* proj_next, void* stream);

size_t eqd_kv_blocks_bytes(int32_t n_nodes);
int eqd_project_tc(const eqd_graph* g, const eqd_layer* p, const float* h , float* proj,
                   void* kv, void* stream);
int eqd_project_tc0(const eqd_graph* g, const eqd_layer* p, const float* h0 , float* proj ,
                    void* kv, float* x5 , void* stream);
int eqd_kv_blocks(const eqd_graph* g, const float* proj, int32_t pw, int32_t koff, int32_t voff, void* kv,
                  void* stream);
int eqd_attention_tc(const eqd_graph* g, const float* proj, const void* kv, float* mu, void* stream);
int eqd_node_mlp_tc(const eqd_graph* g, const eqd_layer* p, const float* h_in, const float* aggr,
                    const float* mu, const float* h0, float* h_out, void* stream);
int eqd_node_stage_tc(const eqd_graph* g, const eqd_layer* p, const eqd_layer* p_next,
                      const float* h_in, const float* h0, const float* proj, const float* aggr, void* kv,
                      float* mu, float* h_out, float* proj_next, void* stream);

int eqd_attention_tc0(const eqd_graph* g, const float* proj , const void* kv, const float* x5 ,
                      float* mu , void* stream);
int eqd_node_mlp_tc0(const eqd_graph* g, const eqd_layer* p, const float* h0 , const float* aggr,
                     const float* mu , float* h_out , void* stream);
int eqd_node_stage_tc0(const eqd_graph* g, const eqd_layer* p, const eqd_layer* p_next, const float* h0,
                       const float* proj, const float* aggr, void* kv, const float* x5, float* mu, float* h_out,
                       float* proj_next, void* stream);

int eqd_iegmn_layer_forward(const eqd_graph* g, const eqd_layer* p, const eqd_layer* p_next,
                            const float* h_in, int32_t ldh, const float* h0,
                            const double* x_in, const double* x_orig,
                            float* proj, float* proj_next, float* aggr, float* mu,
                            float* h_out, double* x_out, int32_t* status, void* stream);

int eqd_head_fold(const eqd_head_params* hp, double* m_qk , void* stream);

int eqd_keypoints(const eqd_graph* g, const eqd_head_params* hp, const float* h ,
                  const double* x , void* workspace, size_t workspace_bytes,
                  double* keypts, double* ymean, double* cov, void* stream);
int eqd_keypoints_dropout(const eqd_graph* g, const eqd_head_params* hp, const eqd_dropout* dropout, const float* h,
                          const double* x, void* workspace, size_t workspace_bytes, double* keypts, double* ymean,
                          double* cov, void* stream);

int eqd_kabsch_apply(const eqd_graph* g, const double* cov, const double* ymean, const float* x_lig_in,
                     const int32_t* pair_mask, float* rot, float* trans, float* ligand_out,
                     double* sing, int32_t* status, void* stream);


typedef struct eqd_forward_io {
  const float* emb;
  const float* res_lig;
  const float* res_rec;
  const float* mu_lig;
  const float* mu_rec;
  const float* x_lig;
  const float* x_rec;
  float* rot;
  float* trans;
  float* ligand_out;
  double* sing;
  int32_t* status;
  float* h_out;
  double* x_out;
  double* keypts;
  double* cov;
  double* ymean;
  void* const* stage_events;
  void* train_stash;
  size_t train_stash_bytes;
} eqd_forward_io;

size_t eqd_forward_workspace_bytes(const eqd_graph* g);
size_t eqd_forward_stash_bytes(const eqd_graph* g, int32_t n_layers);
int eqd_forward_stash_offsets(const eqd_graph* g, int32_t n_layers, size_t* out);
int eqd_iegmn_forward(const eqd_graph* g, const eqd_layer* const* layers, int32_t n_layers,
                      const eqd_head_params* hp, const eqd_forward_io* io, void* workspace, size_t workspace_bytes,
                      void* stream);


size_t eqd_tn_partial_floats(int64_t nrows, int32_t K, int32_t ncols, int32_t* rows_per_chunk_out, int32_t* nchunks_out);
int eqd_tn_gemm(const float* X, int32_t ldx, int32_t K, const float* D, int32_t ldd, int32_t ncols, int64_t nrows,
                float alpha, float* partial, float* colsum, int32_t* nchunks_out, void* stream);
int eqd_grad_reduce(const float* partial, int32_t nchunks, int64_t stride, const int32_t* src_index,
                    const int32_t* dst_index, int32_t n, float* grad, void* stream);

int eqd_bwd_node_mlp(const eqd_graph* g, const eqd_layer* p, const float* w_node1_lin, const float* w_node2_lin,
                     const float* h_in, int32_t ldh, const float* aggr, const float* mu, int32_t ldmu, const float* h0,
                     const float* dh_out, float* dh_in, float* daggr, float* dmu, float* dh0_acc, float* n5_out,
                     float* du_out, float* vec_partial , int32_t* n_partials_out, void* stream);
int eqd_bwd_attention(const eqd_graph* g, const eqd_layer* p, const float* proj, const float* mu, int32_t ldmu,
                      const float* dmu, float* dP, float* rowstat, void* stream);
int eqd_bwd_edge(const eqd_graph* g, const eqd_layer* p, const float* w2lin, const float* w3lin, const float* proj,
                 const double* x_in, const float* daggr, const double* dx_out, float* ein_out, float* n1_out,
                 float* msg_out, float* dz3_out, float* dmsg_out, float* dz1_out, double* dxrel_out,
                 float* vec_partial , int32_t* n_partials_out, void* stream);
int eqd_bwd_edge_gather(const eqd_graph* g, const int32_t* out_ptr, const int32_t* out_edge, const float* dz1,
                        const double* dxrel, const double* dx_out, float eta, float* dP, int32_t ldp, double* dx_in,
                        void* stream);
int eqd_bwd_project(const eqd_graph* g, const eqd_layer* p, const float* w_projT, const float* dP, float* dh,
                    void* stream);
int eqd_bwd_embed(const eqd_graph* g, const float* res_lig, const float* res_rec, const float* dh0_acc,
                  const float* dh_layer0, float* demb, void* stream);
size_t eqd_bwd_head_workspace_bytes(int32_t n_nodes, int32_t n_node_tiles, int32_t n_pairs);
int eqd_bwd_head(const eqd_graph* g, const eqd_head_params* hp, const float* h, const double* x, const double* cov,
                 const float* x_lig_in, const float* dcoors, const double* dkeypts, const float* drot,
                 const float* dtrans, void* workspace, size_t workspace_bytes, float* dh, double* dx, float* dpre,
                 float* g_wkey, float* g_wquery, void* stream);
int eqd_bwd_head_dropout(const eqd_graph* g, const eqd_head_params* hp, const eqd_dropout* dropout, const float* h,
                         const double* x, const double* cov, const float* x_lig_in, const float* dcoors,
                         const double* dkeypts, const float* drot, const float* dtrans, void* workspace,
                         size_t workspace_bytes, float* dh, double* dx, float* dpre, float* g_wkey, float* g_wquery,
                         void* stream);

int eqd_bwd_layer_inputs(const eqd_graph* g, const eqd_layer* p, const float* dz1, const double* dx_out, float* dhe,
                         double* dx_orig, void* stream);
int eqd_bwd_inputs(const eqd_graph* g, const float* dh0_acc, const float* dh_layer0, const float* mu_lig,
                   const float* mu_rec, const double* dx_layer0, const double* dx_orig, const float* rot,
                   const float* dcoors, float* dmu, double* dx, void* stream);

size_t eqd_losses_workspace_bytes(int32_t n_rec_nodes, int32_t n_pocket_total);
int eqd_losses(const eqd_graph* g, const float* pred_lig , const float* bound_lig ,
               const float* bound_rec , const double* keypts ,
               const int32_t* pocket_ptr , const float* pocket_lig, const float* pocket_rec ,
               int32_t n_pocket_total, int32_t max_pocket ,
               float pocket_ot_loss_weight, float intersection_loss_weight,
               float intersection_sigma, float intersection_surface_ct, void* workspace, size_t workspace_bytes,
               double* parts , double* total ,
               float* dcoors , double* dkeypts , int32_t* err_flags, void* stream);

size_t eqd_graph_build_workspace_bytes(int32_t n_nodes);
int eqd_graph_build_knn(int32_t n_prot, int32_t n_nodes, int32_t max_protein_nodes, const int32_t* seg_ptr,
                        const int32_t* atom_ptr, const float* atoms, const float* nca_c, const float* bound_ca, float cutoff,
                        int32_t max_neighbor, void* workspace, size_t workspace_bytes, int32_t* deg, float* x,
                        float* mu_r_norm, void* stream);
int eqd_graph_build_edges(int32_t n_nodes, const int32_t* row_ptr, const int32_t* deg, const void* workspace,
                          int32_t* col_src, int32_t* edge_dst, float* he, void* stream);

typedef struct eqd_pair_archive {
  int32_t n_pairs;
  const int64_t* lig_node_ptr;
  const int64_t* rec_node_ptr;
  const int64_t* lig_edge_ptr;
  const int64_t* rec_edge_ptr;
  const int64_t* pocket_ptr;
  const uint8_t* lig_res_feat;
  const uint8_t* rec_res_feat;
  const float* lig_x;
  const float* rec_x;
  const float* lig_mu_r_norm;
  const float* rec_mu_r_norm;
  const int32_t* lig_src;
  const int32_t* lig_dst;
  const int32_t* rec_src;
  const int32_t* rec_dst;
  const float* lig_he;
  const float* rec_he;
  const float* lig_new_x;
  const float* pocket_coors;
  const float* bound_lig;
  const float* bound_rec;
  const double* lig_centroid;
} eqd_pair_archive;

typedef struct eqd_batch_out {
  float* res_feat;
  float* x;
  float* new_x;
  float* mu_r_norm;
  int32_t* row_ptr;
  int32_t* col_src;
  int32_t* edge_dst;
  float* he_lig;
  float* he_rec;
  int32_t* seg_ptr;
  int32_t* node_tiles;
  int32_t* pocket_ptr;
  float* pocket_lig;
  float* pocket_rec;
  float* bound_lig;
  float* bound_rec;
  double* rot;
  double* trans;
} eqd_batch_out;

int eqd_assemble_batch(const eqd_pair_archive* archive, int32_t n_batch, const int32_t* offsets, int32_t max_segment_edges,
                       uint64_t seed, uint64_t step, int32_t slot0, float translation_interval, int32_t repose,
                       const eqd_batch_out* out, void* stream);

int eqd_rmsd_meter(const eqd_graph* g, const float* lig_pred, const float* rec_pred, const float* lig_true,
                   const float* rec_true, double* out , void* stream);

int eqd_sqnorm_partials(const float* g, int64_t n, double* partial, int32_t n_partial, void* stream);
int eqd_clip_adam(float* w, float* g, float* m, float* v, int64_t n, const double* sq_partial, int32_t n_partial,
                  float max_norm, float lr, float beta1, float beta2, float eps, float weight_decay, int32_t step,
                  float scale_extra, float* norm_out, void* stream);

void* eqd_event_create(void);
void eqd_event_destroy(void* event);
float eqd_event_elapsed_ms(void* begin, void* end);

#ifdef __cplusplus
}
#endif
#endif
```

Baseline: 42690.

## Fold edge message linear layer into node MLP weights to skip a GEMM

```diff
diff --git a/equidock_public_b200/_native.py b/equidock_public_b200/_native.py
--- a/equidock_public_b200/_native.py
+++ b/equidock_public_b200/_native.py
@@ -6,7 +6,7 @@
 _HERE = os.path.dirname(os.path.abspath(__file__))
 LIB_PATH = os.environ.get('EQD_LIB_PATH') or os.path.join(_HERE, 'libeqd_iegmn.so')
 
-ABI_VERSION = 14
+ABI_VERSION = 15
 EDGE_FEATS, N_RBF, HID, H0, H0_PAD, N_RES_TYPES, HEADS, TILE_ROWS = 27, 15, 64, 69, 72, 21, 50, 128
 STATUS_SVD_DEGENERATE, STATUS_NAN, STATUS_DEGREE_OVERFLOW, STATUS_BAD_RESIDUE = 1, 2, 4, 8
 
@@ -49,8 +49,12 @@
     return d
 
 
+class EqdMsgFold(C.Structure):
+    _fields_ = [('w_node_tc', _vp), ('c', _vp)]
+
+
 class EqdLayer(C.Structure):
-    _fields_ = [('dev', EqdLayerParams), ('consts', EqdLayerConsts), ('dropout', EqdDropout)]
+    _fields_ = [('dev', EqdLayerParams), ('consts', EqdLayerConsts), ('dropout', EqdDropout), ('fold', EqdMsgFold)]
 
 
 class EqdForwardIO(C.Structure):
@@ -87,6 +91,7 @@
     'eqd_project': (C.c_int, [_G, _L, _vp, _i32, _vp, _vp]),
     'eqd_edge_stage': (C.c_int, [_G, _L, _vp, _vp, _vp, _vp, _vp, _vp, _vp]),
     'eqd_edge_stage_ffma': (C.c_int, [_G, _L, _vp, _vp, _vp, _vp, _vp, _vp, _vp]),
+    'eqd_edge_stage_fold': (C.c_int, [_G, _L, _vp, _vp, _vp, _vp, _vp, _vp, _vp]),
     'eqd_node_stage': (C.c_int, [_G, _L, _L, _vp, _i32, _vp, _vp, _vp, _vp, _vp, _vp, _vp]),
     'eqd_kv_blocks_bytes': (C.c_size_t, [_i32]),
     'eqd_project_tc': (C.c_int, [_G, _L, _vp, _vp, _vp, _vp]),
@@ -98,6 +103,7 @@
     'eqd_attention_tc': (C.c_int, [_G, _vp, _vp, _vp, _vp]),
     'eqd_node_mlp_tc': (C.c_int, [_G, _L, _vp, _vp, _vp, _vp, _vp, _vp]),
     'eqd_node_stage_tc': (C.c_int, [_G, _L, _L, _vp, _vp, _vp, _vp, _vp, _vp, _vp, _vp, _vp]),
+    'eqd_node_stage_tc_fold': (C.c_int, [_G, _L, _L, _vp, _vp, _vp, _vp, _vp, _vp, _vp, _vp, _vp]),
     'eqd_iegmn_layer_forward': (C.c_int, [_G, _L, _L, _vp, _i32, _vp, _vp, _vp, _vp, _vp, _vp, _vp, _vp, _vp, _vp,
                                           _vp]),
     'eqd_head_fold': (C.c_int, [_H, _vp, _vp]),
diff --git a/equidock_public_b200/csrc/edge_stage_tc.cu b/equidock_public_b200/csrc/edge_stage_tc.cu
--- a/equidock_public_b200/csrc/edge_stage_tc.cu
+++ b/equidock_public_b200/csrc/edge_stage_tc.cu
@@ -37,7 +37,7 @@
   unsigned long long w_bar;
 };
 
-template <int P>
+template <int P, bool FOLD>
 __global__ void __launch_bounds__(TC_THREADS, 1)
 edge_stage_tc_kernel(eqd_graph g, eqd_layer_params p, const __grid_constant__ EdgeConsts cst_p,
                      const float* __restrict__ proj, const double* __restrict__ x_in, const double* __restrict__ x_orig,
@@ -278,6 +278,14 @@
           x1 = fmaf(__fmul_rn(__fadd_rn(x1, -mean[h]), rstd[h]), gj.y, bj.y);
         }
       }
+      if constexpr (FOLD) {
+#pragma unroll
+        for (int j = 0; j < 8; ++j)
+#pragma unroll
+          for (int h = 0; h < 2; ++h)
+            *reinterpret_cast<float2*>(W.msg + (fr0 + 8 * h) * TC_LD + 8 * j + fc) =
+                make_float2(v[4 * j + 2 * h], v[4 * j + 2 * h + 1]);
+      }
       acc_to_a_split3<4, P>(v, af);
     }
     if (has_next) {
@@ -290,9 +298,9 @@
           return b_desc_ex(w_saddr + TC_W23_BASE + sp * TC_W23_SPLIT + kb * 4096 + hn * 1024, 2048, 128); };
       };
       float m[32], hd[32];
-      wg_gemm6_rs_issue<64, 4, 0, false, P>(m, af, w23(0), false);
+      if constexpr (!FOLD) wg_gemm6_rs_issue<64, 4, 0, false, P>(m, af, w23(0), false);
       wg_gemm6_rs_issue<64, 4, 0, false, P>(hd, af, w23(1), false);
-      wg_mma_wait(m);
+      if constexpr (!FOLD) wg_mma_wait(m);
       wg_mma_wait(hd);
       float u[32];
 #pragma unroll
@@ -301,8 +309,10 @@
         const float2 b3 = *reinterpret_cast<const float2*>(&cst.b3[8 * j + fc]);
 #pragma unroll
         for (int h = 0; h < 2; ++h) {
-          *reinterpret_cast<float2*>(W.msg + (fr0 + 8 * h) * TC_LD + 8 * j + fc) =
-              make_float2(__fadd_rn(m[4 * j + 2 * h], b2.x), __fadd_rn(m[4 * j + 2 * h + 1], b2.y));
+          if constexpr (!FOLD) {
+            *reinterpret_cast<float2*>(W.msg + (fr0 + 8 * h) * TC_LD + 8 * j + fc) =
+                make_float2(__fadd_rn(m[4 * j + 2 * h], b2.x), __fadd_rn(m[4 * j + 2 * h + 1], b2.y));
+          }
           const float x0 = __fadd_rn(hd[4 * j + 2 * h], b3.x), x1 = __fadd_rn(hd[4 * j + 2 * h + 1], b3.y);
           u[4 * j + 2 * h] = fmaxf(x0, __fmul_rn(x0, slope));
           u[4 * j + 2 * h + 1] = fmaxf(x1, __fmul_rn(x1, slope));
@@ -386,26 +396,24 @@
   __syncthreads();
 }
 
-template <int P>
+template <int P, bool FOLD>
 static int launch_edge_stage_tc(const eqd_graph* g, const eqd_layer* p_l, const float* proj, const double* x_in,
                                 const double* x_orig, float* aggr, double* x_out, int32_t* status, int tn, void* stream) {
   const int ntiles = (g->n_nodes + tn - 1) / tn;
   EdgeConsts cst;
   memcpy(&cst, p_l->consts.edge, sizeof(cst));
   size_t smem = sizeof(TcSmem) + 128;
-  EQD_SET_SMEM((edge_stage_tc_kernel<P>), smem);
+  EQD_SET_SMEM((edge_stage_tc_kernel<P, FOLD>), smem);
   int grid = (ntiles + TC_WGS - 1) / TC_WGS;
   if (grid > EQD_SMS) grid = EQD_SMS;
-  edge_stage_tc_kernel<P><<<grid, TC_THREADS, smem, (cudaStream_t)stream>>>(*g, p_l->dev, cst, proj, x_in, x_orig, aggr,
-                                                                           x_out, status, tn);
+  edge_stage_tc_kernel<P, FOLD><<<grid, TC_THREADS, smem, (cudaStream_t)stream>>>(*g, p_l->dev, cst, proj, x_in, x_orig,
+                                                                                  aggr, x_out, status, tn);
   EQD_CUDA_LAUNCH_CHECK();
   return EQD_OK;
 }
 
-}
-
-extern "C" int eqd_edge_stage(const eqd_graph* g, const eqd_layer* p_l, const float* proj, const double* x_in,
-                              const double* x_orig, float* aggr, double* x_out, int32_t* status, void* stream) {
+static int edge_stage(const eqd_graph* g, const eqd_layer* p_l, const float* proj, const double* x_in,
+                      const double* x_orig, float* aggr, double* x_out, int32_t* status, void* stream, bool fold) {
   const eqd_layer_params* p = p_l ? &p_l->dev : nullptr;
   if (!g || !p || !proj || !x_in || !x_orig || !aggr || !x_out || !status) return EQD_ERR_BAD_ARG;
   if (!p->w_edge_tc) return EQD_ERR_BAD_ARG;
@@ -416,10 +424,26 @@
   if ((reinterpret_cast<uintptr_t>(g->he_lig) | reinterpret_cast<uintptr_t>(g->he_rec) |
        reinterpret_cast<uintptr_t>(p->w_edge_tc)) & 15)
     return EQD_ERR_BAD_ARG;
-  if (g->max_in_degree > TC_ROWS || p_l->dropout.p > 0.f) return eqd_edge_stage_ffma(g, p_l, proj, x_in, x_orig, aggr, x_out, status, stream);
+  if (g->max_in_degree > TC_ROWS || p_l->dropout.p > 0.f)
+    return fold ? EQD_ERR_UNSUPPORTED : eqd_edge_stage_ffma(g, p_l, proj, x_in, x_orig, aggr, x_out, status, stream);
   if (g->n_nodes <= 0) return EQD_OK;
   int tn = TC_ROWS / g->max_in_degree;
   if (tn > TC_MAX_TN) tn = TC_MAX_TN;
-  return products == 3 ? eqd::launch_edge_stage_tc<3>(g, p_l, proj, x_in, x_orig, aggr, x_out, status, tn, stream)
-                       : eqd::launch_edge_stage_tc<6>(g, p_l, proj, x_in, x_orig, aggr, x_out, status, tn, stream);
-}
+  if (fold)
+    return products == 3 ? launch_edge_stage_tc<3, true>(g, p_l, proj, x_in, x_orig, aggr, x_out, status, tn, stream)
+                         : launch_edge_stage_tc<6, true>(g, p_l, proj, x_in, x_orig, aggr, x_out, status, tn, stream);
+  return products == 3 ? launch_edge_stage_tc<3, false>(g, p_l, proj, x_in, x_orig, aggr, x_out, status, tn, stream)
+                       : launch_edge_stage_tc<6, false>(g, p_l, proj, x_in, x_orig, aggr, x_out, status, tn, stream);
+}
+
+}
+
+extern "C" int eqd_edge_stage(const eqd_graph* g, const eqd_layer* p_l, const float* proj, const double* x_in,
+                              const double* x_orig, float* aggr, double* x_out, int32_t* status, void* stream) {
+  return eqd::edge_stage(g, p_l, proj, x_in, x_orig, aggr, x_out, status, stream, false);
+}
+
+extern "C" int eqd_edge_stage_fold(const eqd_graph* g, const eqd_layer* p_l, const float* proj, const double* x_in,
+                                   const double* x_orig, float* abar, double* x_out, int32_t* status, void* stream) {
+  return eqd::edge_stage(g, p_l, proj, x_in, x_orig, abar, x_out, status, stream, true);
+}
diff --git a/equidock_public_b200/csrc/forward.cu b/equidock_public_b200/csrc/forward.cu
--- a/equidock_public_b200/csrc/forward.cu
+++ b/equidock_public_b200/csrc/forward.cu
@@ -72,6 +72,31 @@
   out[0] = s.h0; out[1] = s.x; out[2] = s.x_stride; out[3] = s.h; out[4] = s.h_stride; out[5] = s.aggr; out[6] = s.a_stride;
   out[7] = s.mu; out[8] = s.m_stride;
   return EQD_OK;
+}
+
+namespace {
+enum NodeStage { NODE_FP32, NODE_TC, NODE_TC0 };
+bool any_dropout(const eqd_layer* const* layers, int n_layers) {
+  for (int li = 0; li < n_layers; ++li)
+    if (layers[li]->dropout.p > 0.f) return true;
+  return false;
+}
+bool tc_layer0(const eqd_layer* const* layers, bool drop) {
+  const eqd_layer_params* l0 = &layers[0]->dev;
+  return l0->dh == EQD_H0 && l0->w_proj_tc && l0->w_node_tc && !drop;
+}
+NodeStage node_stage_of(const eqd_layer* const* layers, int n_layers, int li, bool drop) {
+  const eqd_layer_params* lp = &layers[li]->dev;
+  const eqd_layer_params* lpn = li + 1 < n_layers ? &layers[li + 1]->dev : nullptr;
+  if (lp->dh == EQD_HID && lp->w_node_tc && !drop && (!lpn || lpn->w_proj_tc)) return NODE_TC;
+  if (li == 0 && tc_layer0(layers, drop) && (!lpn || lpn->w_proj_tc)) return NODE_TC0;
+  return NODE_FP32;
+}
+bool folds(const eqd_graph* g, const eqd_layer* const* layers, int n_layers, int li, bool drop, bool stash) {
+  const eqd_layer* l = layers[li];
+  return !stash && l->fold.w_node_tc && l->fold.c && l->dev.w_edge_tc && g->max_in_degree >= 1 &&
+         g->max_in_degree <= 64 && node_stage_of(layers, n_layers, li, drop) == NODE_TC;
+}
 }
 
 extern "C" int eqd_iegmn_forward(const eqd_graph* g, const eqd_layer* const* layers, int32_t n_layers,
@@ -128,10 +153,8 @@
   if (rc) return rc;
   const eqd_layer* l0_l = layers[0];
   const eqd_layer_params* l0 = &l0_l->dev;
-  bool drop = false;
-  for (int li = 0; li < n_layers; ++li) drop = drop || layers[li]->dropout.p > 0.f;
-  const bool tc0 = l0->dh == EQD_H0 && l0->w_proj_tc && l0->w_node_tc && !drop;
-  if (tc0) rc = eqd_project_tc0(g, l0_l, h0, pa, kv, x5, stream);
+  const bool drop = any_dropout(layers, n_layers);
+  if (tc_layer0(layers, drop)) rc = eqd_project_tc0(g, l0_l, h0, pa, kv, x5, stream);
   else rc = eqd_project(g, l0_l, h0, l0->dh == EQD_H0 ? EQD_H0_PAD : EQD_HID, pa, stream);
   if (rc) return rc;
   const float* h_in = h0;
@@ -140,7 +163,6 @@
   for (int li = 0; li < n_layers; ++li) {
     const eqd_layer* lp_l = layers[li];
     const eqd_layer* lpn_l = li + 1 < n_layers ? layers[li + 1] : nullptr;
-    const eqd_layer_params* lp = &lp_l->dev;
     const eqd_layer_params* lpn = lpn_l ? &lpn_l->dev : nullptr;
     const bool last = lpn == nullptr;
     float* h_out = last ? io->h_out : hbuf[li & 1];
@@ -153,14 +175,19 @@
       aggr = reinterpret_cast<float*>(sb + sl.aggr + (size_t)li * sl.a_stride);
       mu = reinterpret_cast<float*>(sb + sl.mu + (size_t)li * sl.m_stride);
     }
+    const bool fold = folds(g, layers, n_layers, li, drop, sb != nullptr);
+    const NodeStage ns = node_stage_of(layers, n_layers, li, drop);
     stage_event(li, 0);
-    rc = eqd_edge_stage(g, lp_l, pa, x_in, x0, aggr, x_out, io->status, stream);
+    rc = fold ? eqd_edge_stage_fold(g, lp_l, pa, x_in, x0, aggr, x_out, io->status, stream)
+              : eqd_edge_stage(g, lp_l, pa, x_in, x0, aggr, x_out, io->status, stream);
     if (rc) return rc;
     stage_event(li, 1);
     stage_event(li, 2);
-    if (lp->dh == EQD_HID && lp->w_node_tc && !drop && (!lpn || lpn->w_proj_tc)) {
+    if (fold) {
+      rc = eqd_node_stage_tc_fold(g, lp_l, lpn_l, h_in, h0, pa, aggr, kv, mu, h_out, pb, stream);
+    } else if (ns == NODE_TC) {
       rc = eqd_node_stage_tc(g, lp_l, lpn_l, h_in, h0, pa, aggr, kv, mu, h_out, pb, stream);
-    } else if (li == 0 && tc0 && (!lpn || lpn->w_proj_tc)) {
+    } else if (ns == NODE_TC0) {
       rc = eqd_node_stage_tc0(g, lp_l, lpn_l, h0, pa, aggr, kv, x5, mu, h_out, pb, stream);
     } else {
       rc = eqd_node_stage(g, lp_l, lpn_l, h_in, ldh, h0, pa, aggr, sb ? mu : nullptr, h_out, pb, stream);
diff --git a/equidock_public_b200/csrc/node_mlp_tc.cu b/equidock_public_b200/csrc/node_mlp_tc.cu
--- a/equidock_public_b200/csrc/node_mlp_tc.cu
+++ b/equidock_public_b200/csrc/node_mlp_tc.cu
@@ -20,11 +20,11 @@
   unsigned long long w_bar;
 };
 
-template <int P>
+template <int P, bool FOLD>
 __global__ void __launch_bounds__(NM_CHAINS * 128, 1)
 node_mlp_tc_kernel(int n_nodes, eqd_layer_params p, const __grid_constant__ NmConsts cst, const float* __restrict__ h_in,
                    const float* __restrict__ aggr, const float* __restrict__ mu, const float* __restrict__ h0,
-                   float* __restrict__ h_out) {
+                   float* __restrict__ h_out, const int* __restrict__ row_ptr, const float* __restrict__ cfold) {
   extern __shared__ __align__(128) unsigned char smem_raw[];
   NmSmem& S = *reinterpret_cast<NmSmem*>(smem_raw);
   const int tid = threadIdx.x, wgi = tid >> 7, t = tid & 127, lane = t & 31;
@@ -65,6 +65,14 @@
       x4[hh] = row < nvalid ? *reinterpret_cast<const float2*>(h0 + (long)(node0 + row) * EQD_H0_PAD + 64 + fc)
                             : make_float2(0.f, 0.f);
     }
+    bool fold_row[2] = {false, false};
+    if constexpr (FOLD) {
+#pragma unroll
+      for (int hh = 0; hh < 2; ++hh) {
+        const int row = fr0 + 8 * hh;
+        fold_row[hh] = row < nvalid && __ldg(row_ptr + node0 + row + 1) > __ldg(row_ptr + node0 + row);
+      }
+    }
     float acc[32], hs[32];
 #pragma unroll
     for (int j = 0; j < 8; ++j) {
@@ -92,6 +100,21 @@
       wg_gemm6_rs_issue<64, 4, 0, false, P>(d, af, [&](int sp, int kb) {
         return b_desc_ex(w_saddr + (4 * pc + kb) * 2048 + sp * NM_W5_SPLIT, 1024, 128); }, false);
       wg_mma_wait(d);
+      if constexpr (FOLD) {
+        if (pc == 1) {
+#pragma unroll
+          for (int j = 0; j < 8; ++j) {
+            const float2 cj = __ldg(reinterpret_cast<const float2*>(cfold + 8 * j + fc));
+#pragma unroll
+            for (int hh = 0; hh < 2; ++hh) {
+              if (fold_row[hh]) {
+                d[4 * j + 2 * hh] = __fadd_rn(d[4 * j + 2 * hh], cj.x);
+                d[4 * j + 2 * hh + 1] = __fadd_rn(d[4 * j + 2 * hh + 1], cj.y);
+              }
+            }
+          }
+        }
+      }
 #pragma unroll
       for (int i = 0; i < 32; ++i) acc[i] = __fadd_rn(acc[i], d[i]);
     }
@@ -354,26 +377,36 @@
   }
 }
 
-template <int P>
+static eqd_layer_params node_params(const eqd_layer* p_l, bool fold) {
+  eqd_layer_params p = p_l->dev;
+  if (fold) p.w_node_tc = p_l->fold.w_node_tc;
+  return p;
+}
+
+template <int P, bool FOLD>
 static int launch_node_mlp_tc(const eqd_graph* g, const eqd_layer* p_l, const float* h_in, const float* aggr,
                               const float* mu, const float* h0, float* h_out, void* stream) {
   NmConsts cst;
   memcpy(&cst, p_l->consts.node, sizeof(cst));
   const int ntiles = (g->n_nodes + 63) / 64;
   const size_t smem = sizeof(NmSmem) + 128;
-  EQD_SET_SMEM(node_mlp_tc_kernel<P>, smem);
+  EQD_SET_SMEM((node_mlp_tc_kernel<P, FOLD>), smem);
   int grid = (ntiles + NM_CHAINS - 1) / NM_CHAINS;
   if (grid > EQD_SMS) grid = EQD_SMS;
-  node_mlp_tc_kernel<P><<<grid, NM_CHAINS * 128, smem, (cudaStream_t)stream>>>(g->n_nodes, p_l->dev, cst, h_in, aggr, mu,
-                                                                             h0, h_out);
+  node_mlp_tc_kernel<P, FOLD><<<grid, NM_CHAINS * 128, smem, (cudaStream_t)stream>>>(
+      g->n_nodes, node_params(p_l, FOLD), cst, h_in, aggr, mu, h0, h_out, FOLD ? g->row_ptr : nullptr,
+      FOLD ? p_l->fold.c : nullptr);
   EQD_CUDA_LAUNCH_CHECK();
   return EQD_OK;
 }
 
-}
-
-extern "C" int eqd_node_mlp_tc(const eqd_graph* g, const eqd_layer* p_l, const float* h_in, const float* aggr,
-                               const float* mu, const float* h0, float* h_out, void* stream) {
+static bool fold_ok(const eqd_layer* p_l) {
+  const eqd_msg_fold& f = p_l->fold;
+  return f.w_node_tc && f.c && !((reinterpret_cast<uintptr_t>(f.w_node_tc) | reinterpret_cast<uintptr_t>(f.c)) & 15);
+}
+
+static int node_mlp_tc(const eqd_graph* g, const eqd_layer* p_l, const float* h_in, const float* aggr, const float* mu,
+                       const float* h0, float* h_out, void* stream, bool fold) {
   const eqd_layer_params* p = p_l ? &p_l->dev : nullptr;
   if (!g || !p || !h_in || !aggr || !mu || !h0 || !h_out) return EQD_ERR_BAD_ARG;
   if (p_l->dropout.p > 0.f) return EQD_ERR_UNSUPPORTED;
@@ -382,9 +415,20 @@
   const int products = eqd_mma_products(p);
   if (!products) return EQD_ERR_UNSUPPORTED;
   if (!p->w_node_tc || (reinterpret_cast<uintptr_t>(p->w_node_tc) & 15)) return EQD_ERR_BAD_ARG;
+  if (fold && (!fold_ok(p_l) || !g->row_ptr)) return EQD_ERR_BAD_ARG;
   if (g->n_nodes <= 0) return EQD_OK;
-  return products == 3 ? eqd::launch_node_mlp_tc<3>(g, p_l, h_in, aggr, mu, h0, h_out, stream)
-                       : eqd::launch_node_mlp_tc<6>(g, p_l, h_in, aggr, mu, h0, h_out, stream);
+  if (fold)
+    return products == 3 ? launch_node_mlp_tc<3, true>(g, p_l, h_in, aggr, mu, h0, h_out, stream)
+                         : launch_node_mlp_tc<6, true>(g, p_l, h_in, aggr, mu, h0, h_out, stream);
+  return products == 3 ? launch_node_mlp_tc<3, false>(g, p_l, h_in, aggr, mu, h0, h_out, stream)
+                       : launch_node_mlp_tc<6, false>(g, p_l, h_in, aggr, mu, h0, h_out, stream);
+}
+
+}
+
+extern "C" int eqd_node_mlp_tc(const eqd_graph* g, const eqd_layer* p_l, const float* h_in, const float* aggr,
+                               const float* mu, const float* h0, float* h_out, void* stream) {
+  return eqd::node_mlp_tc(g, p_l, h_in, aggr, mu, h0, h_out, stream, false);
 }
 
 extern "C" int eqd_node_mlp_tc0(const eqd_graph* g, const eqd_layer* p_l, const float* h0, const float* aggr,
@@ -408,6 +452,29 @@
 }
 
 extern "C" int eqd_attention_tc0(const eqd_graph*, const float*, const void*, const float*, float*, void*);
+extern "C" int eqd_project_tc(const eqd_graph*, const eqd_layer*, const float*, float*, void*, void*);
+int eqd_attention_tc_products(const eqd_graph*, const float*, const void*, float*, int, void*);
+
+namespace eqd {
+
+static int node_stage_tc(const eqd_graph* g, const eqd_layer* p_l, const eqd_layer* p_next_l, const float* h_in,
+                         const float* h0, const float* proj, const float* aggr, void* kv, float* mu, float* h_out,
+                         float* proj_next, void* stream, bool fold) {
+  const eqd_layer_params* p = p_l ? &p_l->dev : nullptr;
+  const eqd_layer_params* p_next = p_next_l ? &p_next_l->dev : nullptr;
+  if (!g || !p || !kv || !mu) return EQD_ERR_BAD_ARG;
+  if (p_next && !proj_next) return EQD_ERR_BAD_ARG;
+  const int products = eqd_mma_products(p);
+  if (!products) return EQD_ERR_UNSUPPORTED;
+  int rc = eqd_attention_tc_products(g, proj, kv, mu, products, stream);
+  if (rc) return rc;
+  rc = node_mlp_tc(g, p_l, h_in, aggr, mu, h0, h_out, stream, fold);
+  if (rc) return rc;
+  if (p_next) rc = eqd_project_tc(g, p_next_l, h_out, proj_next, kv, stream);
+  return rc;
+}
+
+}
 
 extern "C" int eqd_node_stage_tc0(const eqd_graph* g, const eqd_layer* p_l, const eqd_layer* p_next_l,
                                   const float* h0, const float* proj, const float* aggr, void* kv, const float* x5,
@@ -425,23 +492,14 @@
   return rc;
 }
 
-extern "C" int eqd_project_tc(const eqd_graph*, const eqd_layer*, const float*, float*, void*, void*);
-int eqd_attention_tc_products(const eqd_graph*, const float*, const void*, float*, int, void*);
-
-
 extern "C" int eqd_node_stage_tc(const eqd_graph* g, const eqd_layer* p_l, const eqd_layer* p_next_l,
                                  const float* h_in, const float* h0, const float* proj, const float* aggr, void* kv,
                                  float* mu, float* h_out, float* proj_next, void* stream) {
-  const eqd_layer_params* p = p_l ? &p_l->dev : nullptr;
-  const eqd_layer_params* p_next = p_next_l ? &p_next_l->dev : nullptr;
-  if (!g || !p || !kv || !mu) return EQD_ERR_BAD_ARG;
-  if (p_next && !proj_next) return EQD_ERR_BAD_ARG;
-  const int products = eqd_mma_products(p);
-  if (!products) return EQD_ERR_UNSUPPORTED;
-  int rc = eqd_attention_tc_products(g, proj, kv, mu, products, stream);
-  if (rc) return rc;
-  rc = eqd_node_mlp_tc(g, p_l, h_in, aggr, mu, h0, h_out, stream);
-  if (rc) return rc;
-  if (p_next) rc = eqd_project_tc(g, p_next_l, h_out, proj_next, kv, stream);
-  return rc;
-}
+  return eqd::node_stage_tc(g, p_l, p_next_l, h_in, h0, proj, aggr, kv, mu, h_out, proj_next, stream, false);
+}
+
+extern "C" int eqd_node_stage_tc_fold(const eqd_graph* g, const eqd_layer* p_l, const eqd_layer* p_next_l,
+                                      const float* h_in, const float* h0, const float* proj, const float* abar, void* kv,
+                                      float* mu, float* h_out, float* proj_next, void* stream) {
+  return eqd::node_stage_tc(g, p_l, p_next_l, h_in, h0, proj, abar, kv, mu, h_out, proj_next, stream, true);
+}
diff --git a/equidock_public_b200/engine.py b/equidock_public_b200/engine.py
--- a/equidock_public_b200/engine.py
+++ b/equidock_public_b200/engine.py
@@ -70,6 +70,15 @@
     for li, d in enumerate(descs):
         c = nat.EqdLayer.from_buffer_copy(d)
         c.dropout = nat.dropout_descriptor(p, seed, first_layer + li, rank)
+        out.append(c)
+    return out
+
+
+def without_fold(descs):
+    out = []
+    for d in descs:
+        c = nat.EqdLayer.from_buffer_copy(d)
+        c.fold = nat.EqdMsgFold()
         out.append(c)
     return out
 
@@ -134,6 +143,10 @@
             w5p = z(64, 272)
             w5p[:, :261] = w5
             tc['w_node_tc'] = torch.cat([umma_bf16x3(w5p), umma_bf16x3(w6)]).contiguous()
+            w5a = w5[:, 64:128].double()
+            w5p[:, 64:128] = (w5a @ w2d).float()
+            tc['w_node_tc_fold'] = torch.cat([umma_bf16x3(w5p), umma_bf16x3(w6)]).contiguous()
+            tc['c_fold'] = (w5a @ f('edge_mlp.4.bias').double()).float()
             groups = [w1[:, 0:64], w1[:, 64:128], wq, wk, wv]
             tc['w_proj_tc'] = torch.cat([umma_bf16x3(gw.contiguous()) for gw in groups]).contiguous()
             assert tc['w_node_tc'].numel() * 2 == 129024 and tc['w_proj_tc'].numel() * 2 == 122880
@@ -171,7 +184,7 @@
         s = lay.dev
         s.dh, s.dhp = dh, dhp
         for k, v in self.t.items():
-            if not k.startswith('_'):
+            if not k.startswith('_') and k not in ('w_node_tc_fold', 'c_fold'):
                 setattr(s, k, v.data_ptr())
         for name, host in (('edge', self.edge_consts_host), ('node', self.node_consts_host), ('proj_bias', self.proj_bias_host)):
             if host is not None:
@@ -189,6 +202,8 @@
         if src is not self.struct:
             d = nat.EqdLayer.from_buffer_copy(self.struct)
             d.dev.mma_products = mma_products
+            if mma_products == 3:
+                d.fold.w_node_tc, d.fold.c = self.t['w_node_tc_fold'].data_ptr(), self.t['c_fold'].data_ptr()
             self._descriptors[mma_products] = (self.struct, d)
         return d
 
@@ -464,7 +479,7 @@
     def forward(self, plan: GraphPlan, emb: torch.Tensor, layers: List[PackedLayer], head: PackedHead,
                 res_l, res_r, mu_l, mu_r, x_l, x_r, check_status: bool = True, log=None,
                 stage_timer=None, record_event: bool = True, train_stash=None,
-                mma_products: int = 0, dropout=None) -> Dict[str, torch.Tensor]:
+                mma_products: int = 0, dropout=None, fold: bool = True) -> Dict[str, torch.Tensor]:
         with torch.cuda.device(self.device):
             lib, dev = self.lib, self.device
             st = C.c_void_p(torch.cuda.current_stream(dev).cuda_stream)
@@ -494,7 +509,8 @@
                 io.train_stash, io.train_stash_bytes = train_stash.data_ptr(), int(train_stash.numel())
             events = stage_timer.new_forward(len(layers)) if stage_timer is not None else None
             io.stage_events = C.cast(events, C.c_void_p) if events is not None else None
-            descs = with_dropout([l.descriptor(mma_products) for l in layers], dropout)
+            descs = [l.descriptor(mma_products) for l in layers]
+            descs = with_dropout(descs if fold else without_fold(descs), dropout)
             larr = (C.POINTER(nat.EqdLayer) * len(layers))(*[C.pointer(d) for d in descs])
             nat.check(lib.eqd_iegmn_forward(g, larr, len(layers), C.byref(head.struct), C.byref(io), nat.ptr(ws),
                                             plan.forward_ws_bytes, st), 'eqd_iegmn_forward')
diff --git a/include/eqd_iegmn.h b/include/eqd_iegmn.h
--- a/include/eqd_iegmn.h
+++ b/include/eqd_iegmn.h
@@ -8,7 +8,7 @@
 extern "C" {
 #endif
 
-#define EQD_ABI_VERSION 14
+#define EQD_ABI_VERSION 15
 
 #define EQD_EDGE_FEATS 27
 #define EQD_N_RBF 15
@@ -92,10 +92,16 @@
   int32_t reserved;
 } eqd_dropout;
 
+typedef struct eqd_msg_fold {
+  const void* w_node_tc;
+  const float* c;
+} eqd_msg_fold;
+
 typedef struct eqd_layer {
   eqd_layer_params dev;
   eqd_layer_consts consts;
   eqd_dropout dropout;
+  eqd_msg_fold fold;
 } eqd_layer;
 
 typedef struct eqd_head_params {
@@ -129,6 +135,10 @@
 
 int eqd_edge_stage_ffma(const eqd_graph* g, const eqd_layer* p, const float* proj,
                         const double* x_in, const double* x_orig, float* aggr, double* x_out,
+                        int32_t* status , void* stream);
+
+int eqd_edge_stage_fold(const eqd_graph* g, const eqd_layer* p, const float* proj,
+                        const double* x_in, const double* x_orig, float* abar, double* x_out,
                         int32_t* status , void* stream);
 
 int eqd_node_stage(const eqd_graph* g, const eqd_layer* p, const eqd_layer* p_next,
@@ -148,6 +158,9 @@
 int eqd_node_stage_tc(const eqd_graph* g, const eqd_layer* p, const eqd_layer* p_next,
                       const float* h_in, const float* h0, const float* proj, const float* aggr, void* kv,
                       float* mu, float* h_out, float* proj_next, void* stream);
+int eqd_node_stage_tc_fold(const eqd_graph* g, const eqd_layer* p, const eqd_layer* p_next,
+                           const float* h_in, const float* h0, const float* proj, const float* abar, void* kv,
+                           float* mu, float* h_out, float* proj_next, void* stream);
 
 int eqd_attention_tc0(const eqd_graph* g, const float* proj , const void* kv, const float* x5 ,
                       float* mu , void* stream);
@@ -218,6 +231,7 @@
                      const float* h_in, int32_t ldh, const float* aggr, const float* mu, int32_t ldmu, const float* h0,
                      const float* dh_out, float* dh_in, float* daggr, float* dmu, float* dh0_acc, float* n5_out,
                      float* du_out, float* vec_partial , int32_t* n_partials_out, void* stream);
+
 int eqd_bwd_attention(const eqd_graph* g, const eqd_layer* p, const float* proj, const float* mu, int32_t ldmu,
                       const float* dmu, float* dP, float* rowstat, void* stream);
 int eqd_bwd_edge(const eqd_graph* g, const eqd_layer* p, const float* w2lin, const float* w3lin, const float* proj,
```

Result: no change. 42690 (median of 6 runs) (-0.0%).
